# haoyuzhao123/CGRayTracing

Hardware: AMD Instinct MI355X
Metric: Mrays/sec (primary+secondary) at 1920x1080 spp=64 (higher is better)
Workload: dtype f64

## Files before the change

cgraytracing_amd/_capi.py:

```python
from __future__ import annotations

import ctypes as C
import os

import sys

_HERE = os.path.dirname(os.path.abspath(__file__))
CGRT_VERSION = 112
LIB_PATH = os.path.join(_HERE, "libcgrt.so")
if os.environ.get("CGRT_LIB"):
    if os.environ.get("CGRT_DEV_LIBS") == "1":
        LIB_PATH = os.environ["CGRT_LIB"]
        print("cgraytracing_amd: DEVELOPMENT library %s (CGRT_LIB + CGRT_DEV_LIBS=1)" % LIB_PATH, file=sys.stderr)
    else:
        print("cgraytracing_amd: CGRT_LIB ignored (set CGRT_DEV_LIBS=1 to load a development build)", file=sys.stderr)

CGRT_OK = 0
CGRT_NCOUNTERS = 8
CNT_RAYS, CNT_HITPOINTS, CNT_WAVE_ITERS, CNT_NODE_TESTS, CNT_TRI_TESTS = 0, 1, 2, 3, 4


class CgrtError(RuntimeError):
    def __init__(self, code, msg):
        super().__init__("libcgrt error %d: %s" % (code, msg))
        self.code = code


class Camera(C.Structure):
    _fields_ = [("cam", C.c_double * 3), ("half_width", C.c_double), ("focus_plane", C.c_double),
                ("lens_radius", C.c_double)]


class PosedCamera(C.Structure):
    _fields_ = [("base", Camera), ("origin", C.c_double * 3), ("right", C.c_double * 3), ("up", C.c_double * 3),
                ("forward", C.c_double * 3)]


class Grid(C.Structure):
    _fields_ = [("width", C.c_int32), ("height", C.c_int32), ("rows", C.c_int32), ("row_offset", C.c_int32),
                ("stripe_rows", C.c_int32), ("stripe_rank", C.c_int32), ("stripe_nranks", C.c_int32),
                ("spp", C.c_int32), ("sample_offset", C.c_int32), ("spp_total", C.c_int32),
                ("max_depth", C.c_int32), ("flags", C.c_int32), ("seed", C.c_uint64)]


GRID_STATS, GRID_ACCUMULATE, GRID_SPLIT_SAMPLES, GRID_NO_REORDER, GRID_FORCE_REORDER, GRID_HITPOINTS = 1, 2, 4, 8, 16, 32
GRID_NO_TILE_ORDER, GRID_DIFFUSE_TILES, GRID_NO_SPHERE_PAIRS, GRID_NO_SPHERE_MASKS = 64, 128, 256, 512
GRID_SAMPLE_RELAY, GRID_NO_SAMPLE_RELAY, GRID_SAMPLE_RELAY_4 = 1024, 2048, 4096
GRID_RELAY_MIRROR, GRID_RELAY_NO_MIRROR = 8192, 16384
GRID_RELAY_CHUNKS_FIRST, GRID_RELAY_MIRROR_FIRST, GRID_RELAY_INTERLEAVED, GRID_RELAY_ORDER_MASK = 32768, 65536, 98304, 98304
GRID_NO_LENS_STAGE, GRID_NO_SURE_TILES = 131072, 262144
GRID_RELAY_COST_START, GRID_NO_RELAY_COST_START, GRID_RELAY_BOOST, GRID_NO_RELAY_BOOST = 524288, 1048576, 2097152, 4194304
GRID_NO_LENS_TABLE, GRID_LENS_TABLE = 8388608, 16777216
GRID_NO_INSIDE_TRIPS = 33554432
GRID_POSED = 67108864


class Photons(C.Structure):
    _fields_ = [("light", C.c_double * 3), ("jitter", C.c_double), ("power", C.c_double), ("alpha", C.c_double),
                ("nphotons", C.c_int64), ("hashsize", C.c_int32), ("batch", C.c_int32), ("seed", C.c_uint64),
                ("initial_radius", C.c_double), ("pair_cap", C.c_int64)]


class PpmResult(C.Structure):
    _fields_ = [("image", C.c_void_p), ("rgb8", C.c_void_p), ("hp16", C.c_void_p), ("hp_cap", C.c_uint64),
                ("hp_count", C.c_uint64), ("n_events", C.c_uint64), ("n_pairs", C.c_uint64), ("n_batch_halvings", C.c_uint64),
                ("ms_eye", C.c_double),
                ("ms_table", C.c_double), ("ms_photons", C.c_double), ("ms_gather", C.c_double)]


class PpmSessionInfo(C.Structure):
    _fields_ = [("photons_done", C.c_int64), ("hp_count", C.c_uint64), ("n_events", C.c_uint64), ("n_pairs", C.c_uint64),
                ("n_batch_halvings", C.c_uint64), ("device_bytes", C.c_int64), ("ms_eye", C.c_double), ("ms_table", C.c_double),
                ("ms_photons", C.c_double), ("ms_last_add", C.c_double), ("ms_last_image", C.c_double)]


PPM_SESSION_NO_LOOKAHEAD = 1


class SppmSessionInfo(C.Structure):
    _fields_ = [("passes", C.c_int64), ("photons_done", C.c_int64), ("hp_count", C.c_uint64), ("n_events", C.c_uint64),
                ("n_pairs", C.c_uint64), ("n_batch_halvings", C.c_uint64), ("device_bytes", C.c_int64), ("ms_eye", C.c_double),
                ("ms_table", C.c_double), ("ms_photons", C.c_double), ("ms_update", C.c_double)]


class SceneStats(C.Structure):
    _fields_ = [("n_objects", C.c_int32), ("n_spheres", C.c_int32), ("n_planes", C.c_int32),
                ("n_meshes", C.c_int32), ("n_beziers", C.c_int32), ("n_textures", C.c_int32),
                ("n_trees", C.c_int32), ("committed", C.c_int32), ("n_triangles", C.c_int64),
                ("n_nodes", C.c_int64), ("device_bytes", C.c_int64), ("scene_bytes_fp64", C.c_int64)]


class BuildInfo(C.Structure):
    _fields_ = [("mode", C.c_int32), ("n_device_trees", C.c_int32), ("ms_host_build", C.c_double),
                ("ms_device_build", C.c_double), ("ms_commit", C.c_double)]


BUILD_HOST, BUILD_DEVICE = 0, 1


class Rays(C.Structure):
    _fields_ = [("n", C.c_int64), ("org3", C.c_void_p), ("dir3", C.c_void_p), ("keys", C.c_void_p),
                ("first_index", C.c_int64), ("seed", C.c_uint64), ("max_depth", C.c_int32), ("flags", C.c_int32)]


class RayResults(C.Structure):
    _fields_ = [("acc3", C.c_void_p), ("nhit", C.c_void_p), ("hit_obj", C.c_void_p), ("hit_t", C.c_void_p),
                ("hit_normal3", C.c_void_p)]


class HitAttributes(C.Structure):
    _fields_ = [("prim", C.c_void_p), ("uv2", C.c_void_p), ("color3", C.c_void_p), ("material2", C.c_void_p)]


class Occlusion(C.Structure):
    _fields_ = [("tmax", C.c_void_p), ("occluded", C.c_void_p)]


class Bounce(C.Structure):
    _fields_ = [("adj3", C.c_void_p), ("path", C.c_void_p), ("step", C.c_void_p), ("hit_obj", C.c_void_p), ("hit_t", C.c_void_p),
                ("pos3", C.c_void_p), ("normal3", C.c_void_p), ("value3", C.c_void_p), ("child_org3", C.c_void_p),
                ("child_dir3", C.c_void_p), ("child_adj3", C.c_void_p), ("child_path", C.c_void_p), ("child_keys", C.c_void_p),
                ("reserved", C.c_void_p * 2)]


class Wavefront(C.Structure):
    _fields_ = [("max_depth", C.c_int32), ("pad_", C.c_int32), ("min_adj", C.c_double), ("work_bytes", C.c_int64),
                ("acc3", C.c_void_p), ("nhit", C.c_void_p), ("hp9", C.c_void_p), ("hp_ray", C.c_void_p), ("hp_path", C.c_void_p),
                ("hp_cap", C.c_uint64), ("reserved", C.c_void_p * 2)]


WAVEFRONT_MAX_DEPTH = 31


class RayPixels(C.Structure):
    _fields_ = [("width", C.c_int32), ("rows", C.c_int32), ("spp", C.c_int32), ("pad_", C.c_int32), ("pixel", C.c_void_p)]

# ... 55 lines not shown
    "cgrt_ppm_session_create_rays": (C.c_int, [C.c_void_p, C.POINTER(Rays), C.POINTER(RayPixels), C.POINTER(Photons), C.c_int,
                                               C.POINTER(C.c_void_p)]),
    "cgrt_ppm_session_create_hitpoints": (C.c_int, [C.c_void_p, C.POINTER(Hitpoints), C.POINTER(Photons), C.c_int,
                                                    C.POINTER(C.c_void_p)]),
    "cgrt_ppm_session_destroy": (None, [C.c_void_p]),
    "cgrt_ppm_session_add_photons": (C.c_int, [C.c_void_p, C.c_int64]),
    "cgrt_ppm_session_add_photon_rays": (C.c_int, [C.c_void_p, C.POINTER(PhotonRays)]),
    "cgrt_photon_emit": (C.c_int, [C.POINTER(Photons), C.c_int64, C.c_int64, C.c_void_p, C.c_void_p, C.c_void_p, C.c_void_p, C.c_void_p,
                                   C.c_void_p]),
    "cgrt_photon_emit_host": (C.c_int, [C.POINTER(Photons), C.c_int64, C.c_int64, C.c_void_p, C.c_void_p, C.c_void_p, C.c_void_p,
                                        C.c_void_p]),
    "cgrt_photon_ray_events": (C.c_int, [C.c_void_p, C.POINTER(PhotonRays), C.c_uint64, C.c_int64, C.c_int, C.c_void_p, C.c_void_p]),
    "cgrt_ppm_session_image": (C.c_int, [C.c_void_p, C.c_void_p, C.c_void_p]),
    "cgrt_ppm_session_image_device": (C.c_int, [C.c_void_p, C.c_void_p, C.c_void_p, C.c_void_p]),
    "cgrt_ppm_session_hitpoints": (C.c_int, [C.c_void_p, C.c_void_p, C.c_uint64, C.POINTER(C.c_uint64)]),
    "cgrt_ppm_session_get_info": (C.c_int, [C.c_void_p, C.POINTER(PpmSessionInfo)]),
    "cgrt_sppm_session_create": (C.c_int, [C.c_void_p, C.c_int32, C.c_int32, C.c_int32, C.c_int32, C.POINTER(Photons), C.c_int32,
                                           C.POINTER(C.c_void_p)]),
    "cgrt_sppm_session_destroy": (None, [C.c_void_p]),
    "cgrt_sppm_session_pass_grid": (C.c_int, [C.c_void_p, C.POINTER(Camera), C.POINTER(Grid), C.c_int64]),
    "cgrt_sppm_session_pass_rays": (C.c_int, [C.c_void_p, C.POINTER(Rays), C.c_void_p, C.c_int64]),
    "cgrt_sppm_session_image": (C.c_int, [C.c_void_p, C.c_void_p, C.c_void_p]),
    "cgrt_sppm_session_image_device": (C.c_int, [C.c_void_p, C.c_void_p, C.c_void_p, C.c_void_p]),
    "cgrt_sppm_session_pixels": (C.c_int, [C.c_void_p, C.c_void_p]),
    "cgrt_sppm_session_last_hitpoints": (C.c_int, [C.c_void_p, C.c_void_p, C.c_uint64, C.POINTER(C.c_uint64)]),
    "cgrt_sppm_session_get_info": (C.c_int, [C.c_void_p, C.POINTER(SppmSessionInfo)]),
    "cgrt_sppm_update_host": (C.c_int, [C.c_double, C.c_double, C.c_void_p, C.c_double, C.c_void_p, C.c_double, C.c_void_p]),
    "cgrt_sppm_check_host": (C.c_int, [C.c_int32, C.c_int32, C.c_int32, C.c_int32, C.POINTER(Photons), C.c_int32, C.POINTER(Grid)]),
    "cgrt_tonemap_rgb8": (C.c_int, [C.c_int, C.c_void_p, C.c_int, C.c_int, C.c_void_p]),
    "cgrt_write_png": (C.c_int, [C.c_char_p, C.c_int, C.c_int, C.c_void_p]),
    "cgrt_photon_events": (C.c_int, [C.c_void_p, C.POINTER(Photons), C.c_int, C.c_int64, C.c_int32, C.c_void_p,
                                     C.c_void_p]),
    "cgrt_scene_bvh_dump": (C.c_int, [C.c_void_p, C.c_int, C.POINTER(C.c_int32), C.c_void_p, C.c_void_p]),
    "cgrt_scene_bvh_order": (C.c_int, [C.c_void_p, C.c_int, C.POINTER(C.c_int32), C.c_void_p]),
    "cgrt_scene_wide_dump": (C.c_int, [C.c_void_p, C.c_int, C.POINTER(C.c_int32), C.POINTER(C.c_int32), C.c_void_p, C.c_void_p]),
    "cgrt_lens_samples": (C.c_int, [C.c_uint64, C.c_void_p, C.c_void_p, C.c_int, C.c_double, C.c_void_p]),
    "cgrt_surface_colors": (C.c_int, [C.c_void_p, C.c_int, C.c_void_p, C.c_int, C.c_void_p]),
    "cgrt_trace_grid_variant": (C.c_int, [C.c_void_p, C.POINTER(Camera), C.POINTER(Grid), C.c_char_p, C.c_size_t]),
    "cgrt_scene_last_tile_order": (C.c_int, [C.c_void_p, C.c_void_p, C.c_void_p, C.c_void_p, C.c_int64, C.POINTER(C.c_int64)]),
    "cgrt_scene_last_sphere_masks": (C.c_int, [C.c_void_p, C.c_void_p, C.c_int64, C.POINTER(C.c_int64)]),
    "cgrt_scene_last_sure_tiles": (C.c_int, [C.c_void_p, C.c_void_p, C.c_int64, C.POINTER(C.c_int64)]),
    "cgrt_scene_last_sample_relay": (C.c_int, [C.c_void_p, C.POINTER(C.c_int64), C.POINTER(C.c_int32), C.POINTER(C.c_int64)]),
    "cgrt_scene_last_relay_form": (C.c_int, [C.c_void_p, C.POINTER(C.c_int32), C.POINTER(C.c_int32)]),
    "cgrt_scene_last_eye_launches": (C.c_int, [C.c_void_p, C.c_void_p, C.c_int64, C.POINTER(C.c_int64)]),
    "cgrt_relay_start_host": (C.c_int, [C.c_int32, C.c_int32, C.c_int32, C.c_int64, C.c_int32, C.c_int64, C.c_int64, C.c_int64, C.c_void_p,
                                        C.c_void_p, C.c_int32, C.c_int32, C.c_void_p, C.c_int64, C.POINTER(C.c_int64)]),
    "cgrt_scene_last_relay_start": (C.c_int, [C.c_void_p, C.c_void_p, C.c_int64, C.c_void_p, C.c_int64, C.POINTER(C.c_int64),
                                              C.POINTER(C.c_int64), C.POINTER(C.c_int32)]),
    "cgrt_scene_last_relay_boost": (C.c_int, [C.c_void_p, C.POINTER(C.c_int64), C.POINTER(C.c_int32), C.POINTER(C.c_int64), C.POINTER(C.c_uint64),
                                              C.POINTER(C.c_int32), C.POINTER(C.c_int32), C.POINTER(C.c_int32), C.c_void_p, C.c_int64]),
    "cgrt_relay_boost_host": (C.c_int, [C.c_int32, C.c_int32, C.c_int32, C.c_int64, C.c_int32, C.c_int64, C.c_int64, C.c_int64, C.c_void_p,
                                        C.c_void_p, C.c_int32, C.c_int32, C.c_int32, C.c_int32, C.c_int64, C.c_int32, C.c_int32, C.c_int32,
                                        C.c_void_p, C.c_int64, C.c_void_p, C.c_int64, C.POINTER(C.c_int64), C.POINTER(C.c_int64),
                                        C.POINTER(C.c_uint64)]),
    "cgrt_scene_last_lens_stage": (C.c_int, [C.c_void_p, C.POINTER(C.c_int64), C.POINTER(C.c_int64)]),
    "cgrt_scene_last_lens_table": (C.c_int, [C.c_void_p, C.POINTER(C.c_int64), C.POINTER(C.c_int64), C.POINTER(C.c_int32)]),
    "cgrt_scene_last_tile_order_reused": (C.c_int, [C.c_void_p, C.POINTER(C.c_int32)]),
    "cgrt_trace_grid_diffuse_variant": (C.c_int, [C.c_void_p, C.c_void_p, C.c_void_p, C.c_char_p, C.c_size_t]),
    "cgrt_scene_last_diffuse_tiles": (C.c_int, [C.c_void_p, C.POINTER(C.c_int64)]),
    "cgrt_scene_last_inkernel_diffuse_tiles": (C.c_int, [C.c_void_p, C.POINTER(C.c_int64)]),
    "cgrt_trace_rays": (C.c_int, [C.c_void_p, C.POINTER(Rays), C.POINTER(RayResults), C.c_void_p, C.c_void_p]),
    "cgrt_trace_rays_host": (C.c_int, [C.c_void_p, C.POINTER(Rays), C.POINTER(RayResults), C.c_void_p]),
    "cgrt_ray_hit_attributes": (C.c_int, [C.c_void_p, C.POINTER(Rays), C.c_void_p, C.c_void_p, C.POINTER(HitAttributes), C.c_void_p]),
    "cgrt_ray_hit_attributes_host": (C.c_int, [C.c_void_p, C.POINTER(Rays), C.c_void_p, C.c_void_p, C.POINTER(HitAttributes)]),
    "cgrt_trace_rays_variant": (C.c_int, [C.c_void_p, C.POINTER(Rays), C.POINTER(RayResults), C.c_char_p, C.c_size_t]),
    "cgrt_trace_rays_hitpoints": (C.c_int, [C.c_void_p, C.POINTER(Rays), C.c_void_p, C.c_uint64, C.POINTER(C.c_uint64)]),
    "cgrt_occlusion_rays": (C.c_int, [C.c_void_p, C.POINTER(Rays), C.POINTER(Occlusion), C.c_void_p, C.c_void_p]),
    "cgrt_occlusion_rays_host": (C.c_int, [C.c_void_p, C.POINTER(Rays), C.POINTER(Occlusion), C.c_void_p]),
    "cgrt_occlusion_rays_variant": (C.c_int, [C.c_void_p, C.POINTER(Rays), C.c_char_p, C.c_size_t]),
    "cgrt_bounce_rays": (C.c_int, [C.c_void_p, C.POINTER(Rays), C.POINTER(Bounce), C.c_void_p, C.c_void_p]),
    "cgrt_bounce_rays_host": (C.c_int, [C.c_void_p, C.POINTER(Rays), C.POINTER(Bounce), C.c_void_p]),
    "cgrt_bounce_rays_variant": (C.c_int, [C.c_void_p, C.POINTER(Rays), C.c_char_p, C.c_size_t]),
    "cgrt_wavefront_rays": (C.c_int, [C.c_void_p, C.POINTER(Rays), C.POINTER(Wavefront), C.c_void_p, C.POINTER(C.c_uint64), C.c_void_p]),
    "cgrt_wavefront_rays_host": (C.c_int, [C.c_void_p, C.POINTER(Rays), C.POINTER(Wavefront), C.c_void_p, C.POINTER(C.c_uint64)]),
    "cgrt_wavefront_rays_variant": (C.c_int, [C.c_void_p, C.POINTER(Rays), C.c_char_p, C.c_size_t]),
    "cgrt_scene_last_wavefront": (C.c_int, [C.c_void_p, C.POINTER(C.c_int64), C.POINTER(C.c_int64), C.POINTER(C.c_int32)]),
    "cgrt_scene_last_wavefront_rays": (C.c_int, [C.c_void_p, C.c_void_p]),
    "cgrt_camera_rays": (C.c_int, [C.POINTER(Camera), C.POINTER(Grid), C.c_void_p, C.c_void_p, C.c_void_p, C.c_void_p]),
    "cgrt_camera_rays_host": (C.c_int, [C.POINTER(Camera), C.POINTER(Grid), C.c_void_p, C.c_void_p, C.c_void_p]),
    "cgrt_intersect_rays": (C.c_int, [C.c_void_p, C.c_int, C.c_void_p, C.c_void_p, C.c_void_p, C.c_int,
                                      C.c_void_p, C.c_void_p, C.c_void_p]),
    "cgrt_math_probe": (C.c_int, [C.c_int, C.c_int, C.c_void_p, C.c_int64, C.c_void_p]),
    "cgrt_scene_inside_spheres": (C.c_int, [C.c_void_p, C.c_void_p, C.c_void_p, C.c_void_p, C.c_int32, C.POINTER(C.c_int32)]),
    "cgrt_inside_probe": (C.c_int, [C.c_void_p, C.c_int, C.c_void_p, C.c_int64, C.c_void_p]),
}

_lib = None


def lib():
    global _lib
    if _lib is None:
        if not os.path.exists(LIB_PATH):
            raise ImportError(
                "cgraytracing_amd: %s not found -- build the HIP library first "
                "(make -C cgraytracing_amd/csrc, or __graft_entry__.build()). There is no CPU fallback." % LIB_PATH)
        try:
            import torch
        except ImportError:
            pass
        L = C.CDLL(LIB_PATH)
        for name, (res, args) in SIGNATURES.items():
            fn = getattr(L, name)
            fn.restype = res
            fn.argtypes = args
        if L.cgrt_version() != CGRT_VERSION:
            raise ImportError("cgraytracing_amd: %s is ABI version %d, this binding needs %d -- rebuild it (make -C cgraytracing_amd/csrc)"
                              % (LIB_PATH, L.cgrt_version(), CGRT_VERSION))
        _lib = L
    return _lib


def check(rc):
    if rc < 0:
        raise CgrtError(rc, lib().cgrt_last_error().decode("utf-8", "replace"))
    return rc
```

cgraytracing_amd/csrc/cgrt_build.cpp:

```cpp
#include "cgrt_build.h"

#include <algorithm>
#include <atomic>
#include <chrono>
#include <future>
#include <thread>
#include <unordered_map>
#include <cmath>
#include <cstdio>
#include <cstdlib>
#include <cstring>

namespace cgrt {

namespace {

inline double hi3(double a, double b, double c) { return (a > b && a > c) ? a : (b > c ? b : c); }
inline double lo3(double a, double b, double c) { return (a < b && a < c) ? a : (b < c ? b : c); }
inline float round_down(double v) {
    float f = (float)v;
    return ((double)f > v) ? std::nextafterf(f, -INFINITY) : f;
}
inline float round_up(double v) {
    float f = (float)v;
// ... 929 lines not shown
        tr.lenx = t.lenx;
        tr.leny = t.leny;
        tr.isbump = t.isbump ? 1 : 0;
        L.texels.insert(L.texels.end(), t.rgb.begin(), t.rgb.end());
        L.texs.push_back(tr);
    }
    return L;
}

void scene_traits(const HostScene &H, const std::vector<TreeRec> &trees, const CommitKnobs &k, DeviceScene &d) {
    const std::vector<ObjRec> &objs = H.objs;
    d.n_objs = (int32_t)objs.size();
    d.n_lds = std::max(0, std::min({d.n_objs, kLdsObjsMax, k.lds_objs}));
    d.n_trees = (int32_t)trees.size();
    d.n_texs = (int32_t)H.textures.size();
    d.n_beziers = (int32_t)H.beziers.size();
    d.n_cover = (int32_t)(H.cover.size() / 4);
    d.has_wide = 0;
    for (const TreeRec &tr : trees)
        if (tr.nwide > 0) d.has_wide = 1;
    d.has_mesh = trees.empty() ? 0 : 1;
    d.has_bezier = H.beziers.empty() ? 0 : 1;
    d.cached_tree = -1;
    d.cached_nodes = 0;
    for (size_t t = 0; t < trees.size(); t++)
        if (trees[t].nnodes > 0 && trees[t].nnodes <= kNodeCache) {
            d.cached_tree = (int32_t)t;
            d.cached_nodes = trees[t].nnodes;
            break;
        }
    d.all_spheres = 1;
    d.has_glass = 0;
    for (const ObjRec &o : objs) {
        if (o.kind != KIND_SPHERE) d.all_spheres = 0;
        if (!(o.transp < kEps)) d.has_glass = 1;
    }
    {
        int n_mesh = 0, at = -1;
        for (size_t i = 0; i < objs.size(); i++)
            if (objs[i].kind == KIND_MESH) { n_mesh++; at = (int)i; }
        d.prim_obj = -1;
        if (n_mesh == 1 && H.beziers.empty() && objs[(size_t)at].transp < kEps && objs[(size_t)at].tree >= 0 &&
            trees[(size_t)objs[(size_t)at].tree].nwide > 0 && at < d.n_lds)
            d.prim_obj = at;
        d.prim_finish = d.prim_obj >= 0 ? 1 : 0;
        for (const ObjRec &o : objs)
            if (o.kind == KIND_PLANE && o.tree >= 0) d.prim_finish = 0;
    }
    bool planes_plain = true, special = false, plane_trees = false;
    for (const ObjRec &o : objs) {
        const bool diffuse = o.refl < kEps && o.transp < kEps;
        if (o.kind == KIND_PLANE && !diffuse) planes_plain = false;
        if (o.kind == KIND_PLANE && o.tree >= 0) plane_trees = true;
        if (o.kind == KIND_MESH || o.kind == KIND_BEZIER || (o.kind == KIND_SPHERE && !diffuse)) special = true;
    }
    d.light_ok = (planes_plain && special && !d.all_spheres) ? 1 : 0;
    d.single_ray = (planes_plain && !special) ? 1 : 0;
    d.light_trees = plane_trees ? 1 : 0;
    d.light_hf_only = plane_trees ? 1 : 0;
    for (const ObjRec &o : objs)
        if (o.kind == KIND_PLANE && o.tree >= 0 && !(o.transp < kEps && trees[(size_t)o.tree].hfield >= 0)) d.light_hf_only = 0;
    d.prun_begin = d.prun_end = 0;
    if (!k.no_plane_run) {
        auto eligible = [&](int j) { return objs[(size_t)j].kind == KIND_PLANE && objs[(size_t)j].axis >= 0 && objs[(size_t)j].tree < 0; };
        int b = 0;
        while (b < d.n_lds && objs[(size_t)b].kind == KIND_PLANE && !eligible(b)) b++;
        int j = b;
        while (j < d.n_lds && eligible(j)) j++;
        if (j - b >= 3) {
            d.prun_begin = b;
            d.prun_end = j;
        }
    }
    d.inside = InsideTrait{};
    if (d.all_spheres && d.n_objs == d.n_lds && d.n_objs <= kInsideSpheresMax) {
        std::vector<InsideBall> balls;
        std::vector<double> transp;
        for (const ObjRec &o : objs) {
            balls.push_back(InsideBall{{o.a[0], o.a[1], o.a[2]}, o.s0});
            transp.push_back(o.transp);
        }
        d.inside = inside_trait(balls.data(), transp.data(), d.n_objs, true);
    }
}

}
```

cgraytracing_amd/csrc/cgrt_build.h:

```cpp
#ifndef CGRT_BUILD_H
#define CGRT_BUILD_H
#include <cstdint>
#include <string>
#include <vector>

#include "cgrt_types.h"

namespace cgrt {

struct HostTree {
    std::vector<double> tri9;
    std::vector<int32_t> node_lr_size;
    std::vector<double> bbox;
    std::vector<int32_t> leaf_ids;
    std::vector<NodeRec> nodes;
    std::vector<TriRec> tris;
    std::vector<NodeRec> tboxes;
    std::vector<NodeRec> bvh;
    int32_t bvh_nodes = 0;
    bool tri_level = false;
    std::vector<OTriRec> otris;
    std::vector<WideNodeRec> wide;
    int32_t wide_stack = 0;
    void build_bvh(bool opaque);
    bool is_hfield = false;
    HFieldRec hfield{};
    std::vector<HCellRec> hcells;
    std::vector<HCellY> hcell_y;
    void build(bool opaque = false, bool with_bvh = true);
    void build_hfield(int nx, int nz, double x0, double z0, double hx, double hz);
    int dev_kind = 0;
    int64_t dev_ntri = 0;
    int dev_tex = -1;
    double dev_plane_y = 0;
    int dev_obj = -1;
    size_t dev_cover_at = 0;
    int32_t dev_nwide = 0;
    bool dev_balanced = false;
};
int64_t ref_node_count(int64_t n);

struct HostTexture {
    std::vector<uint8_t> rgb;
    int rows = 0, cols = 0;
    double n[3], p[3], lenx = 0, leny = 0;
    bool isbump = false;
};

struct HostScene {
    std::vector<ObjRec> objs;
    std::vector<HostTree> trees;
    std::vector<HostTexture> textures;
    std::vector<BezierRec> beziers;
    std::vector<BezSlabRec> bez_slabs;
    std::vector<double> cover;
    std::string error;
    int build_mode = 0;
    double host_build_ms = 0;

    int add_sphere(const double c[3], double r, const double sc[3], double refl, double transp);
    int add_texture(const uint8_t *rgb, int rows, int cols, const double n[3], const double p[3], double lx,
                    double ly, int isbump);
    int add_plane(const double p[3], const double n[3], const double sc[3], double refl, double transp, int tex);
    int add_mesh_file(const char *file, double a, const double b[3], const double sc[3], double refl,
                      double transp, int type);
    int add_mesh_triangles(const double *tri9, int ntri, const double sc[3], double refl, double transp, int type);
    int add_bezier(const double *cp3, int ncp, const double pos[3], const double sc[3], double refl, double transp);
};

bool load_mesh_file(const char *file, double a, const double b[3], int type, std::vector<double> &tri9,
                    std::string &err);


enum AuxPriority { AUX_LOWEST, AUX_SAME, AUX_HIGH };
struct CommitKnobs {
    bool ref_tree = false;
    int lds_objs = kLdsObjsMax;
    bool no_plane_run = false;
    bool no_bezier_cull = false;
    AuxPriority aux_priority = AUX_LOWEST;
};
CommitKnobs commit_knobs();

float tree_bmax(double max_abs);

struct SceneLayout {
    std::vector<NodeRec> nodes;
    std::vector<TriRec> tris;
    std::vector<OTriRec> otris;
    std::vector<NodeRec> tboxes;
    std::vector<WideNodeRec> wnodes;
    std::vector<HCellRec> hcells;
    std::vector<HCellY> hcell_y;
    std::vector<uint8_t> texels;
    std::vector<TexRec> texs;
    std::vector<HFieldRec> hfields;
    std::vector<TreeRec> trees;
    size_t room_tris = 0, room_otris = 0, room_wnodes = 0, room_hcells = 0;
    int n_dev_trees = 0;
};
SceneLayout scene_layout(const HostScene &H, const CommitKnobs &k);

void scene_traits(const HostScene &H, const std::vector<TreeRec> &trees, const CommitKnobs &k, DeviceScene &d);

}
#endif
```

cgraytracing_amd/csrc/cgrt_eye.hpp:

```cpp
#ifndef CGRT_EYE_HPP
#define CGRT_EYE_HPP
#include "cgrt_lens_stage.h"
#include "cgrt_scene_walk.hpp"
#include "cgrt_sphere_mask.h"
#include "cgrt_sure_first.h"
#include "cgrt_variants.h"

struct Pending {
    V3 o, d, adj;
    int32_t depth_left;
    uint32_t path;
};

#ifndef CGRT_DIFF_WAVES
#define CGRT_DIFF_WAVES 8
#endif
#ifndef CGRT_DIFF_DOF_WAVES
#define CGRT_DIFF_DOF_WAVES 6
#endif
static constexpr int kDiffWaves = CGRT_DIFF_WAVES, kDiffDofWaves = CGRT_DIFF_DOF_WAVES;

__host__ __device__ __forceinline__ void lens_disc(uint64_t k_smp, double &sx, double &sy) {
    uint64_t ctr = k_smp;
    while (true) {
        ctr += kGolden;
        const uint64_t z = fin64(ctr);
        const double ux = div_rand_max((uint32_t)(z >> 33)), uy = div_rand_max((uint32_t)((z >> 2) & 0x7fffffffu));
        sx = ux * 2.0 - 1;
        sy = uy * 2.0 - 1;
        if (sx * sx + sy * sy < 1) break;
    }
}

__device__ __forceinline__ V3 pose_v(const GridParams &g, const V3 &p) {
    V3 w;
    pose_point(g, p.x, p.y, p.z, w.x, w.y, w.z);
    return w;
}

struct HitpointSink {
    double *rec;
    unsigned long long *count;
    unsigned long long cap;
};

template <int NT>
__device__ __forceinline__ bool wave_has_tile(const GridParams &g, int tile_block, int tile_grid) {
    using TG = TileGeom<NT>;
    const int wave = threadIdx.x >> 6;
    const int wtiles_x = (g.W + kWaveTileW - 1) / kWaveTileW, wtiles_y = (g.rows + kWaveTileH - 1) / kWaveTileH;
    int tile_x, tile_y;
    if (tile_grid < 0) {
        const int tiles_x = (g.W + TG::W - 1) / TG::W;
        tile_x = tile_block % tiles_x;
        tile_y = tile_block / tiles_x;
    } else {
        const int tile_blocks = tile_grid / g.chunks;
        if (!tile_of_block(g, tile_block % tile_blocks, tile_x, tile_y, TG::W, TG::H)) return false;
    }
    const int wx = tile_x * (TG::W / kWaveTileW) + (NT == 256 ? (wave & 1) : 0);
    const int wy = tile_y * (TG::H / kWaveTileH) + (NT == 256 ? (wave >> 1) : 0);
    if (!(wx < wtiles_x && wy < wtiles_y)) return false;
    if (g.hidx && g.hidx[wy * wtiles_x + wx] >= 0) return false;
    if (g.light && (g.light[wy * wtiles_x + wx] != 0) != (g.light_mode != 0)) return false;
    return true;
}

struct RelayWg {
    int slot = -1, chunk = 0, s0 = 0, s1 = 0, boost = 0;
};
struct RelayForm {
    unsigned char *area;
    size_t cap;
    int k, slots;
};
template <bool COST>
__device__ __forceinline__ RelayForm relay_form(const GridParams &g, const RelayWg &rw) {
    if (COST && rw.boost) return RelayForm{g.relay + g.relay_boost_off, (size_t)g.boost_cap, g.boost_k, g.boost_slots};
    return RelayForm{g.relay, (size_t)g.relay_cap, g.relay_k, g.relay_slots};
}

template <bool TREES, bool BEZ, bool DOF, bool GLASS, bool SPH, bool STATS, bool HPS, int NT, bool HEAVY, bool SPILL = false, bool HFONLY = false,
          bool DIFF = false, bool PAIR = false, bool PARK = false, bool LSTAGE = false, bool COST = false, bool LTAB = false, bool POSE = false>
__device__ __forceinline__ void trace_grid_body(const DeviceScene &sc, const GridParams &g, float *__restrict__ rgb,
                                                uint32_t *__restrict__ nhit_out, unsigned long long *__restrict__ counters,
                                                const HitpointSink &hps, int tile_block, int tile_grid, const RelayWg rw = RelayWg{},
                                                const uint64_t *__restrict__ lens_row = nullptr) {
    using TG = TileGeom<NT>;
    static_assert(!LTAB || (PAIR && DOF && !LSTAGE), "LTAB: the thin-lens PAIR variants' full and parking bodies");
    static_assert(!PARK || (PAIR && NT == kRelayThreads), "PARK: a relayed tile's later chunks");
    static_assert(!DIFF || (SPH && !GLASS && !HPS && !HEAVY && !STATS && !SPILL), "DIFF: the sphere loop, first hits only");
    static_assert(!PAIR || (SPH && GLASS && !HPS && !HEAVY && !STATS && !SPILL), "PAIR: the glass sphere variants of the tile order");
    static_assert(!LSTAGE || (DIFF && DOF && !PAIR), "LSTAGE: the thin-lens terminal-diffuse body inside a PAIR launch");
    static_assert(!COST || PAIR, "COST: the PAIR variants with a start table");
    static_assert(!POSE || (!DIFF && !PAIR && !LSTAGE && !LTAB), "POSE: no body of the tile order, whose tests stand in the built-in frame");
    static_assert(!LSTAGE || lens_batch_lds(NT) <= (size_t)kLdsLevels * pending_level_bytes(NT), "the lens batches fit the PAIR launch's pending-ray levels");
    const long long tl_t0 = g.timeline ? wall_clock64() : 0;
    if (!HEAVY && !g.timeline) {
        if (!__syncthreads_or((int)wave_has_tile<NT>(g, tile_block, tile_grid))) return;
    }
    constexpr size_t level_bytes = pending_level_bytes(NT), stack_bytes = (size_t)kLdsLevels * level_bytes;
    constexpr bool WALK = TREES && !HFONLY;
    {
        constexpr WgLds chk = wg_lds(wg_ask_trace(NT, TREES, BEZ, GLASS, SPILL, HFONLY), 3, 5, true);
        static_assert(chk.pending == 0 && chk.objs == (GLASS ? stack_bytes : 0) && chk.staging - chk.objs == 3 * sizeof(ObjRec) &&
                          chk.bez - chk.staging == (SPILL ? (NT / 64) * sizeof(ObjRec) : 0) &&
                          chk.nodes - chk.bez == (BEZ ? (NT / 64) * sizeof(BezLds) : 0) &&
                          chk.wstack - chk.nodes == (WALK ? 5 * sizeof(NodeRec) : 0) && chk.has.nodes == WALK &&
                          chk.has.wstack == (WALK && !GLASS && !BEZ),
                      "trace_grid_body's carve-up and cgrt_wg_lds.h");
    }
    extern __shared__ __align__(16) unsigned char lds_raw[];
    ObjRec *lobjs = reinterpret_cast<ObjRec *>(lds_raw + (GLASS ? stack_bytes : 0));
    unsigned char *lrest = reinterpret_cast<unsigned char *>(lobjs + sc.n_lds);
    LdsAux aux;
    if (SPILL) {
        aux.spill = reinterpret_cast<ObjRec *>(lrest) + (threadIdx.x >> 6);
        lrest += (NT / 64) * sizeof(ObjRec);
    }
    aux.bl = BEZ ? reinterpret_cast<volatile BezLds *>(lrest) + (threadIdx.x >> 6) : nullptr;
    if (BEZ) lrest += (NT / 64) * sizeof(BezLds);
    NodeRec *lnodes = reinterpret_cast<NodeRec *>(lrest);
    aux.lnodes = (WALK && sc.cached_tree >= 0) ? lnodes : nullptr;
    aux.wstack = (WALK && !GLASS && !BEZ && sc.has_wide)
                     ? reinterpret_cast<uint2 *>(lrest + ((sc.cached_tree >= 0 ? (size_t)sc.cached_nodes * sizeof(NodeRec) : 0)))
                     : nullptr;
    if (WALK && sc.cached_tree >= 0) {
        const uint4 *src = reinterpret_cast<const uint4 *>(sc.nodes + sc.trees[sc.cached_tree].node_begin);
        uint4 *dst = reinterpret_cast<uint4 *>(lnodes);
        const int n16 = sc.cached_nodes * (int)(sizeof(NodeRec) / 16);
        for (int k = threadIdx.x; k < n16; k += NT) dst[k] = src[k];
    }

    {
        const uint4 *src = reinterpret_cast<const uint4 *>(sc.objs);
        uint4 *dst = reinterpret_cast<uint4 *>(lobjs);
        const int n16 = sc.n_lds * (int)(sizeof(ObjRec) / 16);
        for (int k = threadIdx.x; k < n16; k += NT) dst[k] = src[k];
    }
    __syncthreads();
    const long long cost_t0 = g.probe ? (long long)clock64() : 0;

    const int wave = threadIdx.x >> 6, lane = threadIdx.x & 63;
    const int wtiles_x = (g.W + kWaveTileW - 1) / kWaveTileW, wtiles_y = (g.rows + kWaveTileH - 1) / kWaveTileH;
    const V3 camorg = mk(g.cam[0], g.cam[1], g.cam[2]);
    const V3 camw = POSE ? pose_v(g, camorg) : camorg;
    constexpr bool heavy = HEAVY;
    const unsigned long long lanes_below = (1ull << lane) - 1ull;

    int wx = 0, wy = 0, chunk = 0, s_end = 0;
    bool have_tile = false;
    int w = 0, j = 0, h = 0;
    bool live = false;
    V3 pdir = mk(0, 0, 1), pof = mk(0, 0, 0);
    uint64_t k_pix = 0;
    auto set_pixel = [&](int lx, int ly) {
        w = wx * kWaveTileW + lx;
        j = wy * kWaveTileH + ly;
        h = global_row(g, j);
        live = have_tile && (w < g.W) && (j < g.rows) && (h < g.H);
        const double px = (2.0 * ((double)w / g.W) - 1) * g.half_width;
        const double py = (2.0 * ((double)h / g.H) - 1) * g.half_width * g.H / g.W;
        pdir = normalized(mk(px, py, 0) - camorg);
        pof = pdir * ((g.focus_plane - camorg.z) / pdir.z) + camorg;
        if (POSE) {
            pof = pose_v(g, pof);
            pdir = normalized(pose_v(g, mk(px, py, 0)) - camw);
        }
        k_pix = pixel_key(g.seed, (uint64_t)h * (uint64_t)g.W + (uint64_t)w);
    };
    if (!heavy) {
        const int nb = tile_block;
        int tile_x, tile_y;
        if (tile_grid < 0) {
            const int tiles_x = (g.W + TG::W - 1) / TG::W;
            tile_x = nb % tiles_x;
            tile_y = nb / tiles_x;
        } else {
            const int tile_blocks = tile_grid / g.chunks;
            chunk = nb / tile_blocks;
            if (!tile_of_block(g, nb % tile_blocks, tile_x, tile_y, TG::W, TG::H)) return;
        }
        wx = tile_x * (TG::W / kWaveTileW) + (NT == 256 ? (wave & 1) : 0);
        wy = tile_y * (TG::H / kWaveTileH) + (NT == 256 ? (wave >> 1) : 0);
        have_tile = wx < wtiles_x && wy < wtiles_y;
        if (have_tile && g.hidx && g.hidx[wy * wtiles_x + wx] >= 0) have_tile = false;
        if (have_tile && g.light && (g.light[wy * wtiles_x + wx] != 0) != (g.light_mode != 0)) have_tile = false;
        s_end = (g.chunks > 1) ? ((chunk + 1) * g.chunk_spp < g.spp ? (chunk + 1) * g.chunk_spp : g.spp) : (PAIR && rw.slot >= 0 ? rw.s1 : g.spp);
        set_pixel(lane & 15, lane >> 4);
    }
    const bool masked = DIFF && g.wmask != nullptr;
    uint32_t smask = 0u;
    if (masked) {
        smask = load_uniform(g.wmask + __builtin_amdgcn_readfirstlane(have_tile ? wy * wtiles_x + wx : 0));
        if (sc.n_lds < 32) smask &= (1u << sc.n_lds) - 1u;
    }
    uint32_t sure = (uint32_t)kSureNone;
    if (DIFF && g.wsure != nullptr && have_tile) {
        const uint32_t wt = (uint32_t)__builtin_amdgcn_readfirstlane(wy * wtiles_x + wx);
        sure = (load_uniform(reinterpret_cast<const uint32_t *>(g.wsure) + (wt >> 2)) >> ((wt & 3u) * 8u)) & 0xffu;
        if (sure >= (uint32_t)sc.n_lds) sure = (uint32_t)kSureNone;
    }
    uint64_t k_smp = 0;

    double acc_r = 0, acc_g = 0, acc_b = 0;
    uint32_t my_hits = 0, my_rays = 0, my_nodes = 0, my_tris = 0, wave_iters = 0;
    uint32_t hp_seq = 0;

    Pending deep[2];
    Pending sib;
    bool sib_valid = false;
    unsigned char *lslot = lds_raw;
    int sp = 0;
    int s = (g.chunks > 1) ? chunk * g.chunk_spp : (PAIR && rw.slot >= 0 ? rw.s0 : 0);
    double *park = nullptr;
    uint32_t park_n = 0;
    if (PARK) {
        const RelayForm rf = relay_form<COST>(g, rw);
        park = reinterpret_cast<double *>(rf.area + relay_layout(rf.cap, rf.k, rf.slots).rvals) +
               ((size_t)rw.slot * (size_t)(rf.k - 1) + (size_t)(rw.chunk - 1)) * (size_t)rf.slots * (3 * NT) + threadIdx.x;
    }
    bool have = false;
    V3 o = camorg, d = pdir, adj = mk(1, 1, 1);
    int depth_left = 0;
    uint32_t path = 1;
    int unit_next = 0, unit_end = 0, hrank = 0;
    int unit_pix = 0, unit_smp = 0, unit_rank = 0;
    bool unit_open = false;
    constexpr bool PRE = HEAVY && TREES && !BEZ && !STATS && !SPILL;
    bool pre_valid = false;
    double pre_len = 0;
    int32_t pre_tri = -1;

    const bool staging = LSTAGE && g.lens_batch != 0;
    uint64_t *const lens_slot = reinterpret_cast<uint64_t *>(lrest) + threadIdx.x;
    static_assert(lens_slot_at(1, 0, NT) == NT * sizeof(uint64_t) && lens_slot_at(0, 1, NT) == sizeof(uint64_t), "lens_slot's strides");
    int batch_first = 0, batch_end = 0;
    auto stage_lens = [&](int first, int count) {
        uint32_t rejected = 0u;
        for (int b = 0; b < count; b++) {
            const LensSlot a = lens_stage_first(k_pix, (uint64_t)(g.sample_offset + first + b));
            lens_slot[b * NT] = a.v;
            rejected |= a.done ? 0u : (1u << b);
        }
        if (!live) rejected = 0u;
        while (__ballot(rejected != 0u) != 0ull) {
            if (rejected != 0u) {
                const int b = __ffs((int)rejected) - 1;
                const LensSlot a = lens_stage_retry(lens_slot[b * NT]);
                lens_slot[b * NT] = a.v;
                if (a.done) rejected &= rejected - 1u;
            }
        }
        batch_first = first;
        batch_end = first + count;
    };
    uint64_t z_next = 0;
    if (LTAB && s < s_end) z_next = lens_row[(uint32_t)s * (uint32_t)NT + threadIdx.x];
    auto start_sample = [&](int smp) {
        if (LTAB) {
            double sx, sy;
            lens_point(z_next, sx, sy);
            o = camorg + mk(sx, sy, 0) * g.lens_radius;
            d = normalized(pof - o);
            k_smp = 0;
            if (smp + 1 < s_end) z_next = lens_row[(uint32_t)(smp + 1) * (uint32_t)NT + threadIdx.x];
        } else if (LSTAGE && staging) {
            double sx, sy;
            lens_point(lens_slot[(smp - batch_first) * NT], sx, sy);
            o = camorg + mk(sx, sy, 0) * g.lens_radius;
            d = normalized(pof - o);
            k_smp = 0;
        } else if (DOF) {
            k_smp = sample_key(k_pix, (uint64_t)(g.sample_offset + smp));
            double sx, sy;
            lens_disc(k_smp, sx, sy);
            o = camorg + mk(sx, sy, 0) * g.lens_radius;
            if (POSE) o = pose_v(g, o);
            d = normalized(pof - o);
        } else {
            k_smp = sample_key(k_pix, (uint64_t)(g.sample_offset + smp));
            o = POSE ? camw : camorg;
            d = pdir;
// ... 395 lines not shown
        for (int off = 32; off > 0; off >>= 1) {
            r += __shfl_xor(r, off);
            hh += __shfl_xor(hh, off);
            if (STATS) {
                nn += __shfl_xor(nn, off);
                tt += __shfl_xor(tt, off);
            }
        }
        if (lane == 0 && (r | (unsigned long long)wave_iters) != 0ull) {
            atomicAdd(&counters[CGRT_CNT_RAYS], r);
            atomicAdd(&counters[CGRT_CNT_HITPOINTS], hh);
            atomicAdd(&counters[CGRT_CNT_WAVE_ITERS], (unsigned long long)wave_iters);
            if (STATS) {
                atomicAdd(&counters[CGRT_CNT_NODE_TESTS], nn);
                atomicAdd(&counters[CGRT_CNT_TRI_TESTS], tt);
            }
        }
    }
}

__device__ __forceinline__ unsigned long long *wg_counters_begin(unsigned long long *wg, const unsigned long long *counters) {
    if (!counters) return nullptr;
    if (threadIdx.x < CGRT_NCOUNTERS) wg[threadIdx.x] = 0ull;
    __syncthreads();
    return wg;
}
__device__ __forceinline__ void wg_counters_end(const unsigned long long *wg, unsigned long long *counters) {
    if (!counters) return;
    __syncthreads();
    if (threadIdx.x < CGRT_NCOUNTERS && wg[threadIdx.x] != 0ull) atomicAdd(&counters[threadIdx.x], wg[threadIdx.x]);
}

template <bool TREES, bool BEZ, bool DOF, bool GLASS, bool SPH, bool STATS, bool HPS = false, int NT = 256, bool SPILL = false, bool HFONLY = false,
          bool DIFF = false, bool PAIR = false, bool START = false, bool LTAB = false, bool POSE = false>
__global__ __launch_bounds__(NT, DIFF ? (DOF ? kDiffDofWaves : kDiffWaves) : BEZ ? kBezWaves : ((TREES && !HFONLY) ? kTreeWaves : 4)) void trace_grid_kernel(DeviceScene sc, GridParams g, float *__restrict__ rgb,
                                                             uint32_t *__restrict__ nhit_out,
                                                             unsigned long long *__restrict__ counters,
                                                             HitpointSink hps = HitpointSink{nullptr, nullptr, 0}) {
    int tile_block = (int)blockIdx.x, tile_grid = (int)gridDim.x;
    unsigned entry = blockIdx.x;
    RelayWg rw;
    if (!POSE && g.tile_order) {
        if (g.tile_order == kOrderFull || g.tile_order == kOrderDiffuse) {
            const unsigned first_diffuse = load_uniform(g.plan + 3);
            if (g.tile_order == kOrderDiffuse) entry += first_diffuse;
            if (g.tile_order == kOrderDiffuse ? entry >= load_uniform(g.plan + kOrderClasses) : entry >= first_diffuse) return;
        } else if (PAIR && g.relay_k > 1) {
            const unsigned n_tiles = load_uniform(g.plan + kOrderClasses);
            const unsigned n01 = load_uniform(g.plan + 2), n012 = load_uniform(g.plan + 3);
            RelayBlock rb{n_tiles, 0, false};
            bool tabled = false;
            unsigned b = blockIdx.x, bslot = 0u;
            if (START && g.relay_start_at != 0u) {
                const unsigned n_split = relay_split_entries(n01, n012, (unsigned)g.relay_cap, g.relay_extent);
                const unsigned t0 = n012 + ((unsigned)g.relay_k - 1u) * n_split;
                const unsigned items = g.relay_boost_at != 0u ? load_uniform(g.plan + g.relay_boost_at + kBoostItems) : t0;
                tabled = b < items;
                if (tabled) {
                    rb = relay_start_block(load_uniform(g.plan + g.relay_start_at + b), n_split);
                    if (g.relay_boost_at != 0u && rb.split) bslot = load_uniform(g.plan + g.relay_boost_at + kBoostHead + rb.entry);
                    if (rb.chunk >= (bslot != 0u ? g.boost_k : g.relay_k) || bslot > (unsigned)g.boost_cap) return;
                } else {
                    b -= items - t0;
                }
            }
            if (!tabled) rb = relay_block_ordered(b, (unsigned)g.relay_k, n01, n012, n_tiles, (unsigned)g.relay_cap, g.relay_extent, g.relay_order);
            entry = rb.entry;
            if (entry >= n_tiles) return;
            if (rb.split) {
                const int cs = START && bslot != 0u ? g.boost_chunk_spp : g.relay_chunk_spp;
                rw.slot = START && bslot != 0u ? (int)(bslot - 1u) : (int)entry;
                rw.boost = START && bslot != 0u ? 1 : 0;
                rw.chunk = rb.chunk;
                rw.s0 = relay_first_sample(rb.chunk, cs);
                rw.s1 = relay_end_sample(rb.chunk, cs, g.spp);
            }
        }
        tile_block = (int)load_uniform(g.border + entry);
        tile_grid = -1;
    }
    __shared__ unsigned long long wg_cnt[CGRT_NCOUNTERS];
    unsigned long long *wc = wg_counters_begin(wg_cnt, counters);
    if (PAIR && g.tile_order == kOrderAllDiffuse && entry >= load_uniform(g.plan + 3))
        trace_grid_body<false, false, DOF, false, true, false, false, NT, false, false, false, true, false, false, DOF>(sc, g, rgb, nhit_out, wc, hps, tile_block, tile_grid);
    else if (LTAB && g.lens_table != nullptr && entry < (unsigned)g.lens_table_cap && entry < load_uniform(g.plan + 3)) {
        const uint64_t *lens_row = g.lens_table + (size_t)entry * (size_t)g.lens_table_spp * NT;
        if (rw.chunk > 0)
            trace_grid_body<TREES, BEZ, DOF, GLASS, SPH, STATS, HPS, NT, false, SPILL, HFONLY, DIFF, PAIR, PAIR, false, START, LTAB>(sc, g, rgb, nhit_out, wc, hps, tile_block, tile_grid, rw, lens_row);
        else
            trace_grid_body<TREES, BEZ, DOF, GLASS, SPH, STATS, HPS, NT, false, SPILL, HFONLY, DIFF, PAIR, false, false, START, LTAB>(sc, g, rgb, nhit_out, wc, hps, tile_block, tile_grid, rw, lens_row);
    } else if (PAIR && rw.chunk > 0)
        trace_grid_body<TREES, BEZ, DOF, GLASS, SPH, STATS, HPS, NT, false, SPILL, HFONLY, DIFF, PAIR, PAIR, false, START>(sc, g, rgb, nhit_out, wc, hps, tile_block, tile_grid, rw);
    else
        trace_grid_body<TREES, BEZ, DOF, GLASS, SPH, STATS, HPS, NT, false, SPILL, HFONLY, DIFF, PAIR, false, false, START, false, POSE>(sc, g, rgb, nhit_out, wc, hps, tile_block, tile_grid, rw);
    wg_counters_end(wg_cnt, counters);
}
template <bool TREES, bool BEZ, bool DOF, bool GLASS, bool SPH, bool STATS, int NT = 256, bool POSE = false>
__global__ __launch_bounds__(NT, BEZ ? kBezWaves : (TREES ? kSchedTreeWaves : 4)) void trace_grid_sched_kernel(DeviceScene sc, GridParams g,
                                                                                         float *__restrict__ rgb,
                                                                                         uint32_t *__restrict__ nhit_out,
                                                                                         unsigned long long *__restrict__ counters) {
    const HitpointSink none{nullptr, nullptr, 0};
    const bool heavy_first = (int)blockIdx.x < g.heavy_blocks;
    __shared__ unsigned long long wg_cnt[CGRT_NCOUNTERS];
    unsigned long long *wc = wg_counters_begin(wg_cnt, counters);
    if (NT == 64) {
        if (heavy_first)
            trace_grid_body<TREES, BEZ, DOF, GLASS, SPH, STATS, false, NT, true, false, false, false, false, false, false, false, false, POSE>(sc, g, rgb, nhit_out, wc, none, 0, 1);
        else
            trace_grid_body<TREES, BEZ, DOF, GLASS, SPH, STATS, false, NT, false, false, false, false, false, false, false, false, false, POSE>(
                sc, g, rgb, nhit_out, wc, none, (int)blockIdx.x - g.heavy_blocks, (int)gridDim.x - g.heavy_blocks);
        wg_counters_end(wg_cnt, counters);
        return;
    }
    const bool queued = g.border != nullptr;
    __shared__ unsigned tile_entry;
    for (int phase = 0; phase < 2; phase++) {
        if ((phase == 0) == heavy_first) {
            if (queued || heavy_first)
                trace_grid_body<TREES, BEZ, DOF, GLASS, SPH, STATS, false, NT, true, false, false, false, false, false, false, false, false, POSE>(sc, g, rgb, nhit_out, wc, none, 0, 1);
        } else {
            const unsigned n_entries = queued ? load_uniform(g.plan + 3) : (heavy_first ? 0u : 1u);
            unsigned served = 0;
            while (true) {
                unsigned e = served++;
                if (queued) {
                    __syncthreads();
                    if (threadIdx.x == 0) tile_entry = atomicAdd(&g.plan[4], 1u);
                    __syncthreads();
                    e = tile_entry;
                }
                if (e >= n_entries) break;
                trace_grid_body<TREES, BEZ, DOF, GLASS, SPH, STATS, false, NT, false, false, false, false, false, false, false, false, false, POSE>(
                    sc, g, rgb, nhit_out, wc, none, queued ? (int)g.border[e] : (int)blockIdx.x - g.heavy_blocks,
                    queued ? -1 : (int)gridDim.x - g.heavy_blocks);
            }
        }
    }
    wg_counters_end(wg_cnt, counters);
}

__global__ void finalize_chunks_kernel(GridParams g, float *__restrict__ rgb, uint32_t *__restrict__ nhit_out) {
    const size_t npx = (size_t)g.rows * g.W;
    const size_t px = (size_t)blockIdx.x * blockDim.x + threadIdx.x;
    if (px >= npx) return;
    if (g.hidx) {
        const int wtiles_x = (g.W + kWaveTileW - 1) / kWaveTileW;
        if (g.hidx[(int)((px / g.W) / kWaveTileH) * wtiles_x + (int)((px % g.W) / kWaveTileW)] >= 0) return;
    }
    double r = 0, gg = 0, b = 0;
    uint32_t hits = 0;
    for (int c = 0; c < g.chunks; c++) {
        const size_t q = (size_t)c * npx + px;
        r += g.partial[3 * q + 0];
        gg += g.partial[3 * q + 1];
        b += g.partial[3 * q + 2];
        if (g.partial_nhit) hits += g.partial_nhit[q];
    }
    const float fr = (float)(r * g.inv_spp_total), fg = (float)(gg * g.inv_spp_total), fb = (float)(b * g.inv_spp_total);
    float *dst = rgb + 3 * px;
    if (g.accumulate) {
        dst[0] += fr; dst[1] += fg; dst[2] += fb;
    } else {
        dst[0] = fr; dst[1] = fg; dst[2] = fb;
    }
    if (nhit_out) nhit_out[px] = hits;
}
// ... 431 lines not shown
            }
        }
    }
    const float fr = (float)(r * g.inv_spp_total), fg = (float)(gg * g.inv_spp_total), fb = (float)(b * g.inv_spp_total);
    float *dst = rgb + ((size_t)j * g.W + w) * 3;
    if (g.accumulate) {
        dst[0] += fr; dst[1] += fg; dst[2] += fb;
    } else {
        dst[0] = fr; dst[1] = fg; dst[2] = fb;
    }
    if (nhit_out) nhit_out[(size_t)j * g.W + w] = hits;
}

__global__ void intersect_rays_kernel(DeviceScene sc, int obj, const double *__restrict__ org,
                                      const double *__restrict__ dir, const unsigned long long *__restrict__ keys,
                                      int n, int32_t *__restrict__ hit,
                                      double *__restrict__ len, double *__restrict__ nrm) {
    __shared__ BezLds bl;
    const int i = blockIdx.x * blockDim.x + threadIdx.x;
    const bool on = i < n;
    const int ii = on ? i : 0;
    uint32_t a = 0, b = 0;
    const V3 o = ld3(org + 3 * ii), d = ld3(dir + 3 * ii);
    DeviceScene one = sc;
    one.prun_begin = one.prun_end = 0;
    RayKey rk{keys ? keys[ii] : 0ull, 1, true, 0u};
    const LdsAux aux{&bl, nullptr};
    SceneHit h = intersect_scene<true, true, false, false>(sc.objs + obj, 1, 1, one, o, d, rk, on, aux, a, b);
    if (!on) return;
    hit[i] = h.id >= 0 ? 1 : 0;
    len[i] = h.t;
    nrm[3 * i] = h.n.x;
    nrm[3 * i + 1] = h.n.y;
    nrm[3 * i + 2] = h.n.z;
}

__device__ __forceinline__ V3 surface_color(const DeviceScene &sc, const ObjRec &ob, V3 P) {
    V3 f = ld3(ob.col);
    if (ob.kind == KIND_PLANE && ob.tex >= 0) {
        V3 c;
        if (texture_color(sc.texs[ob.tex], sc.texels, P, c)) f = c;
    }
    return f;
}

__global__ void surface_colors_kernel(DeviceScene sc, int obj, const double *__restrict__ pts, int n, double *__restrict__ out) {
    const int i = blockIdx.x * blockDim.x + threadIdx.x;
    if (i >= n) return;
    const V3 f = surface_color(sc, sc.objs[obj], ld3(pts + 3 * i));
    out[3 * i] = f.x;
    out[3 * i + 1] = f.y;
    out[3 * i + 2] = f.z;
}

__global__ void math_probe_kernel(int op, const double *__restrict__ in, long long n, double *__restrict__ out) {
    const long long i = (long long)blockIdx.x * blockDim.x + threadIdx.x;
    if (i >= n) return;
    if (op == CGRT_PROBE_SQRT) {
        out[i] = sqrt_cr(in[i]);
    } else if (op == CGRT_PROBE_NORMALIZED) {
        const V3 v = normalized(ld3(in + 3 * i));
        out[3 * i] = v.x;
        out[3 * i + 1] = v.y;
        out[3 * i + 2] = v.z;
    } else if (op == CGRT_PROBE_SPHERE_LEN) {
        const double *p = in + 10 * i;
        out[i] = sphere_len(ld3(p), p[3], ld3(p + 4), ld3(p + 7));
    } else {
        const double *p = in + 14 * i;
        sphere_len_pair(ld3(p), p[3], ld3(p + 4), p[7], ld3(p + 8), ld3(p + 11), out[2 * i], out[2 * i + 1]);
    }
}

__global__ void inside_loop_probe_kernel(DeviceScene sc, InsideTrait guarded, const double *__restrict__ in, long long n, double *__restrict__ out) {
    const long long i = (long long)blockIdx.x * blockDim.x + threadIdx.x;
    if (i >= n) return;
    const V3 o = ld3(in + 6 * i), d = ld3(in + 6 * i + 3);
    RayKey rk{0, 1, false, 0u};
    LdsAux aux;
    aux.bl = nullptr;
    aux.lnodes = nullptr;
    uint32_t nn = 0, nt = 0;
    sc.inside = InsideTrait{};
    const SceneHit a = intersect_scene<false, false, true, false, false, false, false, false, true>(sc.objs, sc.n_lds, sc.n_objs, sc, o, d, rk, true, aux, nn, nt);
    sc.inside = guarded;
    const SceneHit b = intersect_scene<false, false, true, false, false, false, false, false, true>(sc.objs, sc.n_lds, sc.n_objs, sc, o, d, rk, true, aux, nn, nt);
    bool took = false;
    for (int k = 0; k < kInsideMax && k < guarded.n && !took; k++)
        took = __ballot(!starts_inside(o, ld3(sc.objs[guarded.idx[k]].a), guarded.rin2[k])) == 0ull;
    out[5 * i] = a.t;
    out[5 * i + 1] = (double)a.id;
    out[5 * i + 2] = b.t;
    out[5 * i + 3] = (double)b.id;
    out[5 * i + 4] = took ? 1.0 : 0.0;
}

#endif
```

cgraytracing_amd/csrc/cgrt_frame.h:

```cpp
#ifndef CGRT_FRAME_H
#define CGRT_FRAME_H
#include <algorithm>
#include <cmath>
#include <cstddef>
#include <cstdint>
#include <cstdio>
#include <cstdlib>
#include <string>

#include "../../include/cgrt.h"
#include "cgrt_lens_stage.h"
#include "cgrt_relay.h"

struct GridParams {
    int32_t W, H, rows, row_offset, stripe_rows, stripe_rank, stripe_nranks;
    int32_t spp, sample_offset, max_depth;
    int32_t accumulate;
    int32_t xcd_tiles;
    int32_t chunks, chunk_spp;
    double *partial;
    uint32_t *partial_nhit;
    const unsigned char *light;
    int32_t light_mode, tile_order;
    const uint32_t *wmask;
    const uint32_t *order;
    const uint32_t *border;
    uint32_t *cost;
    const int32_t *hidx;
    uint32_t *plan;
    double *dvals;
    unsigned char *dcnt;
    double *pconst;
    int32_t probe, heavy_blocks, items_per_tile, units_per_item, maxhp;
    const double *prim_len;
    const int32_t *prim_tri;
    int32_t prim_obj;
    int32_t prim_done;
    int32_t pw_refill, pw_rounds;
    unsigned long long *timeline;
    double inv_spp_total;
    uint64_t seed;
    double cam[3], half_width, focus_plane, lens_radius;
    unsigned char *relay;
    int32_t relay_k, relay_chunk_spp, relay_cap, relay_slots;
    int32_t relay_extent, relay_order;
    int32_t lens_batch;
    uint32_t relay_start_at;
    const unsigned char *wsure;
    uint64_t relay_boost_off;
    uint32_t relay_boost_at;
    int32_t boost_k, boost_chunk_spp, boost_cap, boost_slots, pad_boost_;
    const uint64_t *lens_table;
    int32_t lens_table_cap, lens_table_spp;
    double pose_origin[3], pose_right[3], pose_up[3], pose_forward[3];
    int32_t posed, pad_pose_;
};
static_assert(sizeof(GridParams) == 488, "GridParams is a kernel argument: its layout is fixed");
static_assert(offsetof(GridParams, pose_origin) == 384, "the pose is appended: no earlier field moves");

#if defined(__HIPCC__)
#define CGRT_HD __host__ __device__ __forceinline__
#else
#define CGRT_HD inline
#endif
CGRT_HD void pose_point(const GridParams &g, double x, double y, double z, double &wx, double &wy, double &wz) {
    wx = ((g.pose_origin[0] + g.pose_right[0] * x) + g.pose_up[0] * y) + g.pose_forward[0] * z;
    wy = ((g.pose_origin[1] + g.pose_right[1] * x) + g.pose_up[1] * y) + g.pose_forward[1] * z;
    wz = ((g.pose_origin[2] + g.pose_right[2] * x) + g.pose_up[2] * y) + g.pose_forward[2] * z;
}

static constexpr double kPoseTol = 1e-9;
inline const char *pose_error(const cgrt_camera *cam, const cgrt_grid *grid) {
    if (!(grid->flags & CGRT_GRID_POSED)) return nullptr;
    const cgrt_posed_camera *pc = reinterpret_cast<const cgrt_posed_camera *>(cam);
    const double *ax[3] = {pc->right, pc->up, pc->forward};
    for (int k = 0; k < 3; k++) {
        if (!std::isfinite(pc->origin[k])) return "posed camera: origin is not finite";
        for (int a = 0; a < 3; a++)
            if (!std::isfinite(ax[a][k])) return "posed camera: a basis vector is not finite";
    }
    const auto dot3 = [](const double *a, const double *b) { return a[0] * b[0] + a[1] * b[1] + a[2] * b[2]; };
    for (int a = 0; a < 3; a++)
        if (!(std::fabs(std::sqrt(dot3(ax[a], ax[a])) - 1.0) <= kPoseTol)) return "posed camera: right, up and forward must have length 1 (within 1e-9)";
    for (int a = 0; a < 3; a++)
        if (!(std::fabs(dot3(ax[a], ax[(a + 1) % 3])) <= kPoseTol)) return "posed camera: right, up and forward must be orthogonal (dot products within 1e-9)";
    return nullptr;
}

inline const char *look_at_camera(const double eye[3], const double target[3], const double up_hint[3], double fov_x_deg,
                                  double focus_distance, double lens_radius, cgrt_posed_camera *out) {
    for (int k = 0; k < 3; k++)
        if (!std::isfinite(eye[k]) || !std::isfinite(target[k]) || !std::isfinite(up_hint[k])) return "cgrt_look_at: eye, target and up_hint must be finite";
    if (!(fov_x_deg > 0 && fov_x_deg < 180)) return "cgrt_look_at: fov_x_deg must lie in (0, 180)";
    if (!(focus_distance > 0) || !std::isfinite(focus_distance)) return "cgrt_look_at: focus_distance must be positive";
    if (!(lens_radius >= 0) || !std::isfinite(lens_radius)) return "cgrt_look_at: lens_radius must be >= 0";
// ... 98 lines not shown
            r += cam.lens_radius * std::max(std::fabs(1 - s_lo), std::fabs(1 - s_hi));
        }
        const double vx = sp.s[i][0] - cam.cam[0], vy = sp.s[i][1] - cam.cam[1], vz = sp.s[i][2] - cam.cam[2];
        if (!(std::sqrt(vx * vx + vy * vy + vz * vz) > r)) return true;
    }
    return false;
}
static constexpr int kWaveTileW = 16, kWaveTileH = 4;
static constexpr int kXcds = 8, kSuperW = 4, kSuperH = 4, kSuperTiles = kSuperW * kSuperH;

inline int tile_grid_blocks(int W, int rows, bool xcd_tiles, int tile_w = kTileW, int tile_h = kTileH) {
    const int tiles_x = (W + tile_w - 1) / tile_w, tiles_y = (rows + tile_h - 1) / tile_h;
    if (!xcd_tiles) return tiles_x * tiles_y;
    const int sx = (tiles_x + kSuperW - 1) / kSuperW, sy = (tiles_y + kSuperH - 1) / kSuperH;
    const int nsuper = sx * sy;
    return ((nsuper + kXcds - 1) / kXcds) * kXcds * kSuperTiles;
}

inline GridParams grid_params(const cgrt_camera *cam, const cgrt_grid *grid) {
    GridParams g{};
    g.W = grid->width;
    g.H = grid->height;
    g.rows = grid->rows;
    g.row_offset = grid->row_offset;
    g.stripe_rows = grid->stripe_rows;
    g.stripe_rank = grid->stripe_rank;
    g.stripe_nranks = grid->stripe_nranks;
    g.spp = grid->spp;
    g.sample_offset = grid->sample_offset;
    g.max_depth = grid->max_depth;
    g.accumulate = (grid->flags & CGRT_GRID_ACCUMULATE) ? 1 : 0;
    g.inv_spp_total = 1.0 / (double)grid->spp_total;
    g.seed = grid->seed;
    for (int k = 0; k < 3; k++) g.cam[k] = cam->cam[k];
    g.half_width = cam->half_width;
    g.focus_plane = cam->focus_plane;
    g.lens_radius = cam->lens_radius;
    g.chunks = 1;
    g.chunk_spp = grid->spp;
    g.items_per_tile = 1;
    g.units_per_item = 256;
    g.maxhp = 16;
    g.prim_obj = -1;
    g.pw_refill = 16;
    g.pw_rounds = 8;
    g.pose_right[0] = g.pose_up[1] = g.pose_forward[2] = 1.0;
    if (grid->flags & CGRT_GRID_POSED) {
        const cgrt_posed_camera *pc = reinterpret_cast<const cgrt_posed_camera *>(cam);
        for (int k = 0; k < 3; k++) {
            g.pose_origin[k] = pc->origin[k];
            g.pose_right[k] = pc->right[k];
            g.pose_up[k] = pc->up[k];
            g.pose_forward[k] = pc->forward[k];
        }
        g.posed = 1;
    }
    return g;
}

struct EyeKnobs {
    bool force_reorder = false;
    long long defer_bytes = 0;
    int heavy_div = 32, units_per_item = 256;
    bool no_primwalk = false, pw_no_finish = false;
    int pw_refill = 16, pw_rounds = 8;
    int lds_pad = 0;
    bool no_hfonly = false, no_tile_queue = false, plan_dump = false;
    bool no_sure_tiles = false;
    bool no_order_reuse = false;
    int relay_chunks = kRelayDefaultChunks;
    long long relay_tiles = 0;
    int relay_mirror = -1;
    int relay_order = -1;
    int relay_start = -1;
    int relay_probe_spp = kRelayProbeSpp;
    bool relay_boost_off = false;
    uint32_t relay_boost_num = kRelayBoostNum, relay_boost_den = kRelayBoostDen;
    long long relay_boost_tiles = -1;
    int lens_stage = -1;
    int lens_table = -1;
    long long lens_table_bytes = 0;
    bool lens_table_bytes_set = false;
    bool no_inside_trips = false;
    const char *timeline_file = nullptr;
};
inline const char *env_str(const char *name) { const char *e = std::getenv(name); return e ? e : ""; }
inline bool env_on(const char *name) { const char *e = env_str(name); return *e && *e != '0'; }
inline int env_positive(const char *name, int def) { const int v = std::atoi(env_str(name)); return v > 0 ? v : def; }
inline int relay_order_named(const char *e) {
    const std::string v(e);
    if (v == "chunks_first" || v == "0") return kRelayChunksFirst;
    if (v == "mirror_first" || v == "1") return kRelayMirrorFirst;
    if (v == "interleaved" || v == "2") return kRelayInterleaved;
    return -1;
}
inline int relay_start_named(const char *e) {
    const std::string v(e);
    if (v == "list" || v == "0") return kRelayStartList;
    if (v == "cost" || v == "1") return kRelayStartCost;
    return -1;
}
inline bool relay_boost_named(const char *e, bool &off, uint32_t &num, uint32_t &den) {
    const std::string v(e);
    if (v.empty()) return true;
    if (v == "off" || v == "0") {
        off = true;
        return true;
    }
    const size_t slash = v.find('/');
    if (slash == std::string::npos || slash == 0 || slash + 1 >= v.size()) return false;
    for (size_t i = 0; i < v.size(); i++)
        if (i != slash && (v[i] < '0' || v[i] > '9')) return false;
    if (slash > 6 || v.size() - slash - 1 > 6) return false;
    const unsigned long n = std::strtoul(v.c_str(), nullptr, 10), d = std::strtoul(v.c_str() + slash + 1, nullptr, 10);
    if (n > kRelayBoostMaxTerm || d < 1 || d > kRelayBoostMaxTerm) return false;
    num = (uint32_t)n;
    den = (uint32_t)d;
    return true;
}
static constexpr int kLensStageOff = 0, kLensStageLds = 1;
static constexpr int kLensStageDefault = kLensStageLds;
inline int lens_stage_named(const char *e) {
    const std::string v(e);
    if (v == "off" || v == "0") return kLensStageOff;
    if (v == "lds" || v == "1") return kLensStageLds;
    return -1;
}
static constexpr bool kLensTableAlways = false;
inline int lens_table_named(const char *e) {
    const std::string v(e);
    if (v == "off" || v == "0") return 0;
    if (v == "on" || v == "1") return 1;
    return -1;
}
inline EyeKnobs eye_knobs() {
    static const EyeKnobs once = [] {
        EyeKnobs k;
        k.force_reorder = env_on("CGRT_FORCE_REORDER");
        k.defer_bytes = std::atoll(env_str("CGRT_DEFER_BYTES"));
        k.heavy_div = env_positive("CGRT_HEAVY_DIV", 32);
        k.units_per_item = (env_positive("CGRT_UNITS_PER_ITEM", 256) + 63) / 64 * 64;
        k.no_primwalk = env_on("CGRT_NO_PRIMWALK");
        k.pw_no_finish = env_on("CGRT_PW_NO_FINISH");
        k.pw_refill = env_positive("CGRT_PW_REFILL", 16);
        k.pw_rounds = env_positive("CGRT_PW_ROUNDS", 8);
        k.lds_pad = std::atoi(env_str("CGRT_LDS_PAD"));
        k.no_hfonly = env_on("CGRT_NO_HFONLY");
        k.no_tile_queue = env_on("CGRT_NO_TILE_QUEUE");
        k.plan_dump = env_on("CGRT_PLAN_DUMP");
        k.no_order_reuse = env_on("CGRT_NO_ORDER_REUSE");
        k.no_sure_tiles = env_on("CGRT_NO_SURE_TILES");
        k.relay_chunks = std::min(std::max(env_positive("CGRT_RELAY_CHUNKS", kRelayDefaultChunks), 2), kRelayMaxChunks);
        k.relay_tiles = std::atoll(env_str("CGRT_RELAY_TILES"));
        if (*env_str("CGRT_RELAY_MIRROR")) k.relay_mirror = env_on("CGRT_RELAY_MIRROR") ? 1 : 0;
        k.relay_order = relay_order_named(env_str("CGRT_RELAY_ORDER"));
        k.relay_start = relay_start_named(env_str("CGRT_RELAY_START"));
        if (k.relay_start < 0 && *env_str("CGRT_RELAY_START"))
            std::fprintf(stderr, "cgrt: CGRT_RELAY_START=%s names no start order of this library (list, cost): the default is used\n", env_str("CGRT_RELAY_START"));
        {
            const int ps = std::atoi(env_str("CGRT_RELAY_PROBE_SPP"));
            if (ps == 1 || ps == 2 || ps == 4) k.relay_probe_spp = ps;
        }
        k.lens_stage = lens_stage_named(env_str("CGRT_LENS_STAGE"));
        if (k.lens_stage < 0 && *env_str("CGRT_LENS_STAGE"))
            std::fprintf(stderr, "cgrt: CGRT_LENS_STAGE=%s names no form of this library (off, lds): the default is used\n", env_str("CGRT_LENS_STAGE"));
        k.lens_table = lens_table_named(env_str("CGRT_LENS_TABLE"));
        if (k.lens_table < 0 && *env_str("CGRT_LENS_TABLE"))
            std::fprintf(stderr, "cgrt: CGRT_LENS_TABLE=%s is neither off nor on: the default is used\n", env_str("CGRT_LENS_TABLE"));
        if (*env_str("CGRT_LENS_TABLE_BYTES")) {
            k.lens_table_bytes = std::max(std::atoll(env_str("CGRT_LENS_TABLE_BYTES")), 0ll);
            k.lens_table_bytes_set = true;
        }
        {
            const std::string v(env_str("CGRT_INSIDE_TRIPS"));
            k.no_inside_trips = v == "off" || v == "0";
            if (!v.empty() && !k.no_inside_trips && v != "on" && v != "1")
                std::fprintf(stderr, "cgrt: CGRT_INSIDE_TRIPS=%s is neither off nor on: the default is used\n", v.c_str());
        }
        return k;
    }();
    EyeKnobs k = once;
    k.timeline_file = *env_str("CGRT_TIMELINE_FILE") ? env_str("CGRT_TIMELINE_FILE") : nullptr;
    if (!relay_boost_named(env_str("CGRT_RELAY_BOOST"), k.relay_boost_off, k.relay_boost_num, k.relay_boost_den)) {
        static bool said = false;
        if (!said)
            std::fprintf(stderr, "cgrt: CGRT_RELAY_BOOST=%s is neither off nor a threshold num/den (integers, num <= %u, 1 <= den <= %u): the default is used\n",
                         env_str("CGRT_RELAY_BOOST"), kRelayBoostMaxTerm, kRelayBoostMaxTerm);
        said = true;
    }
    if (*env_str("CGRT_RELAY_BOOST_TILES")) k.relay_boost_tiles = std::max(std::atoll(env_str("CGRT_RELAY_BOOST_TILES")), 0ll);
    return k;
}

struct FrameInputs {
    cgrt_grid grid;
    cgrt_camera cam;
    bool sched, spill, stats, glass;
    int nt;
    bool has_mesh, has_bezier, prim_finish, light_ok;
    int prim_obj;
    EyeKnobs knobs;
    size_t mem_total;
    int n_cu, waves_per_simd;
    bool image = false, sph = false, pair = false;
    bool order_ok = false, aux_stream = false, all_spheres = false;
    int n_objs = 0, n_lds = 0;
    bool all_special = false;
    bool posed = false;
    cgrt_posed_camera posed_cam{};
};

struct ScratchLayout {
    Region partial{}, partial_nhit{}, cost{}, order{}, hidx{}, border{}, plan{}, light{}, dvals{}, dcnt{}, pconst{}, prim_len{}, prim_tri{};
    size_t total = 0;
    void place(GridParams &g, unsigned char *base, bool nhit) const {
        g.partial = partial.in<double>(base);
        g.partial_nhit = nhit ? partial_nhit.in<uint32_t>(base) : nullptr;
        g.cost = cost.in<uint32_t>(base);
        g.order = order.in<uint32_t>(base);
        g.hidx = hidx.in<int32_t>(base);
        g.border = border.in<uint32_t>(base);
        g.plan = plan.in<uint32_t>(base);
        g.light = light.in<unsigned char>(base);
        g.dvals = dvals.in<double>(base);
        g.dcnt = dcnt.in<unsigned char>(base);
        g.pconst = pconst.in<double>(base);
        g.prim_len = prim_len.in<double>(base);
        g.prim_tri = prim_tri.in<int32_t>(base);
    }
};

struct TileOrderPlan {
    bool on = false;
    enum Class3 { None, SecondLaunch, InKernel } class3 = None;
    bool masks = false;
    bool sure = false;
    int lens_stage = kLensStageOff;
    size_t lens_table_cap = 0, lens_table_bytes = 0;
    bool lens_table_always = false;
};

inline bool relay_engaged(int32_t flags, int32_t spp, size_t n_tiles, int n_cu) {
    if ((flags & CGRT_GRID_NO_SAMPLE_RELAY) || spp < 2 * kRelayMinChunkSpp) return false;
    return (flags & CGRT_GRID_SAMPLE_RELAY) || n_tiles >= (size_t)4 * (size_t)n_cu;
}

static constexpr int kRelayDefaultExtent = kRelayMirror, kRelayDefaultOrder = kRelayInterleaved;
struct RelayRule { int extent, order, start; bool boost; };
inline RelayRule relay_rule(int32_t f, const EyeKnobs &kn) {
    const bool asked = (f & CGRT_GRID_SAMPLE_RELAY) != 0;
    const int32_t order_flag = f & CGRT_GRID_RELAY_ORDER_MASK;
    const bool measured = !asked && !order_flag && kn.relay_order < 0;
    const bool names_start = (f & (CGRT_GRID_NO_RELAY_COST_START | CGRT_GRID_RELAY_COST_START)) || kn.relay_start >= 0;
    RelayRule r;
    r.extent = (f & CGRT_GRID_RELAY_MIRROR) ? kRelayMirror : (f & CGRT_GRID_RELAY_NO_MIRROR) ? kRelayGlass
               : kn.relay_mirror >= 0 ? (kn.relay_mirror ? kRelayMirror : kRelayGlass) : asked ? kRelayGlass : kRelayDefaultExtent;
    r.order = order_flag ? (order_flag == CGRT_GRID_RELAY_MIRROR_FIRST ? kRelayMirrorFirst : order_flag == CGRT_GRID_RELAY_INTERLEAVED ? kRelayInterleaved : kRelayChunksFirst)
              : kn.relay_order >= 0 ? kn.relay_order : asked ? kRelayChunksFirst : kRelayDefaultOrder;
    r.start = (f & CGRT_GRID_NO_RELAY_COST_START) ? kRelayStartList : (f & CGRT_GRID_RELAY_COST_START) ? kRelayStartCost
              : kn.relay_start >= 0 ? kn.relay_start : measured ? kRelayStartCost : kRelayStartList;
    r.boost = (f & CGRT_GRID_NO_RELAY_BOOST) ? false : (f & CGRT_GRID_RELAY_BOOST) ? true : !kn.relay_boost_off && !names_start && measured;
    return r;
}

struct RelayArea {
    int k = 0, chunk_spp = 0, slots = 0;
    size_t cap = 0, bytes = 0;
};
static constexpr int kRelayWgPerCu = 4;
struct RelayPlan {
    RelayArea base{1, 0, 0, 0, 0}, boost;
    int spp = 0, extent = kRelayGlass, order = kRelayChunksFirst;
    int start = kRelayStartList, probe_spp = 0;
    size_t start_words = 0, boost_words = 0;
    uint32_t num = 0, den = 1;
    int wg_slots = 0;
    bool relays() const { return base.k > 1; }
    bool boosts() const { return boost.k > base.k; }
    size_t boost_at() const { return align256(base.bytes); }
    size_t bytes() const { return boosts() ? boost_at() + boost.bytes : base.bytes; }
    size_t grid(size_t n_tiles, bool boosted) const { return relay_grid(n_tiles, base.k, base.cap) + (boosted ? boost_words : 0); }
    RelayBoost boost_rule() const {
        return boosts() ? RelayBoost{(uint32_t)boost.k, (uint32_t)boost.cap, boost.chunk_spp, num, den, (uint32_t)wg_slots} : RelayBoost{};
    }
    RelayItems items(uint32_t n01, uint32_t n012, uint32_t n_tiles) const {
        return RelayItems{(uint32_t)base.k, n01, n012, n_tiles, (uint32_t)base.cap, extent, base.chunk_spp, spp};
    }
    TileOrderLayout order_layout(size_t n_tiles, size_t n_wt, bool sure) const {
        return tile_order_layout(n_tiles, n_wt, sure, start_words, boost_words, base.cap, boost.k);
    }
    void place(GridParams &g, unsigned char *buf) const {
        g.relay = buf;
        g.relay_k = base.k;
        g.relay_chunk_spp = base.chunk_spp;
        g.relay_cap = (int32_t)base.cap;
        g.relay_slots = base.slots;
        g.relay_extent = extent;
        g.relay_order = order;
        if (!boosts()) return;
        g.relay_boost_off = boost_at();
        g.boost_k = boost.k;
        g.boost_chunk_spp = boost.chunk_spp;
        g.boost_cap = (int32_t)boost.cap;
        g.boost_slots = boost.slots;
    }
};
inline RelayPlan relay_plan(const cgrt_grid &gr, const EyeKnobs &kn, size_t n_tiles, int n_cu, size_t mem_total) {
    RelayPlan r;
    if (!relay_engaged(gr.flags, gr.spp, n_tiles, n_cu)) return r;
    const auto area = [&gr](const RelayChunks &c, size_t tiles, size_t budget, long long bound) {
        RelayArea a{c.k, c.chunk_spp, relay_slots(c.chunk_spp, gr.max_depth), 0, 0};
        a.cap = relay_cap(tiles, a.k, a.slots, budget, bound);
        a.bytes = relay_layout(a.cap, a.k, a.slots).total;
        return a;
    };
    const RelayChunks rc = relay_chunks(gr.spp, (gr.flags & CGRT_GRID_SAMPLE_RELAY_4) ? kRelayMaxChunks : kn.relay_chunks);
    const RelayArea base = rc.k > 1 ? area(rc, n_tiles, relay_budget(mem_total), kn.relay_tiles) : RelayArea{};
    if (base.cap == 0) return r;
    const RelayRule f = relay_rule(gr.flags, kn);
    r.base = base;
    r.spp = gr.spp, r.extent = f.extent, r.order = f.order;
    r.start = n_tiles < kRelayStartMaxTiles ? f.start : kRelayStartList;
    if (r.start != kRelayStartCost) return r;
    r.probe_spp = std::min(kn.relay_probe_spp, (int)gr.spp);
    r.start_words = relay_start_words(n_tiles, base.k, base.cap);
    const RelayChunks rb = relay_chunks(gr.spp, kRelayMaxChunks);
    if (rb.k <= rc.k || !f.boost || kn.relay_boost_tiles == 0) return r;
    const RelayArea boost = area(rb, base.cap, relay_boost_budget(mem_total, r.boost_at()), kn.relay_boost_tiles);
    if (boost.cap == 0) return r;
    r.boost = boost;
    r.boost_words = relay_boost_extra(base.k, boost.k, boost.cap);
    r.num = kn.relay_boost_num, r.den = kn.relay_boost_den;
    r.wg_slots = n_cu * kRelayWgPerCu;
    return r;
}

struct FramePlan {
    int chunks = 1, chunk_spp = 0;
    bool xcd_tiles = false;
    int maxhp = 1;
    int tile_blocks = 0;
    size_t grid_dim = 0;
    int wtiles_x = 0, wtiles_y = 0;
    size_t n_wt = 0, tile_bytes = 0, kmax = 0;
    bool use_prim = false;
    bool split_light = false, tile_queue = false, prim_done = false;
    int wave_slots = 0, items_per_tile = 1, heavy_blocks = 0;
    unsigned long long plan_div = 0;
    ScratchLayout scratch;
    TileOrderPlan order;
    RelayPlan relay;
};

inline FramePlan frame_plan(const FrameInputs &in, size_t kmax) {
    const cgrt_grid &gr = in.grid;
    const EyeKnobs &kn = in.knobs;
    FramePlan p;
    p.chunk_spp = gr.spp;
    p.xcd_tiles = !in.spill && in.has_mesh && !in.has_bezier;
    p.maxhp = in.glass ? 16 : 1;
    const size_t npx = (size_t)gr.rows * gr.width;
    if ((gr.flags & CGRT_GRID_SPLIT_SAMPLES) && gr.spp >= 32 && !in.spill) {
        int chunks = std::min(gr.spp / 16, 16);
        while (chunks > 1 && (size_t)chunks * npx * 28 > ((size_t)4 << 30)) chunks--;
        if (chunks > 1) {
            p.chunk_spp = (gr.spp + chunks - 1) / chunks;
            p.chunks = (gr.spp + p.chunk_spp - 1) / p.chunk_spp;
        }
    }
    const bool one_wave = in.nt == 64;
    const int waves_per_block = in.nt / 64;
    p.tile_blocks = one_wave ? tile_grid_blocks(gr.width, gr.rows, false, kWaveTileW, kWaveTileH)
                             : tile_grid_blocks(gr.width, gr.rows, p.xcd_tiles);
    p.grid_dim = (size_t)p.tile_blocks * p.chunks;
    TileOrderPlan &o = p.order;
    const bool split_asked = (gr.flags & CGRT_GRID_SPLIT_SAMPLES) != 0;
    o.on = in.image && p.chunks == 1 && !p.xcd_tiles && in.nt == kThreads && in.order_ok && !(gr.flags & CGRT_GRID_NO_TILE_ORDER) && !in.posed;
    if (o.on && !in.all_special) {
        if (in.sph && !in.spill && !in.stats && in.aux_stream && (gr.flags & CGRT_GRID_DIFFUSE_TILES) && !split_asked && !kn.timeline_file)
            o.class3 = TileOrderPlan::SecondLaunch;
        else if (in.pair)
            o.class3 = TileOrderPlan::InKernel;
    }
    o.masks = o.class3 != TileOrderPlan::None && in.all_spheres && in.n_objs <= kSphereMaskMax && in.n_objs == in.n_lds &&
              !(gr.flags & CGRT_GRID_NO_SPHERE_MASKS);
    o.sure = o.masks && !(gr.flags & CGRT_GRID_NO_SURE_TILES) && !kn.no_sure_tiles;
    if (o.class3 == TileOrderPlan::InKernel && in.cam.lens_radius > 0 && !(gr.flags & CGRT_GRID_NO_LENS_STAGE))
        o.lens_stage = kn.lens_stage >= 0 ? kn.lens_stage : kLensStageDefault;
    if (o.on && in.pair && o.class3 != TileOrderPlan::SecondLaunch && !split_asked)
        p.relay = relay_plan(gr, kn, (size_t)p.tile_blocks, in.n_cu, in.mem_total);
    const int lens_table = (gr.flags & CGRT_GRID_NO_LENS_TABLE) ? 0 : (gr.flags & CGRT_GRID_LENS_TABLE) ? 1 : kn.lens_table;
    if (o.on && in.pair && o.class3 != TileOrderPlan::SecondLaunch && !split_asked && in.cam.lens_radius > 0 && lens_table != 0) {
        const size_t budget = kn.lens_table_bytes_set ? (size_t)kn.lens_table_bytes : kLensTableBudget;
        o.lens_table_cap = lens_table_cap((size_t)p.tile_blocks, gr.spp, kThreads, budget);
        o.lens_table_bytes = lens_table_bytes(o.lens_table_cap, gr.spp, kThreads);
        o.lens_table_always = o.lens_table_cap > 0 && (lens_table > 0 || kLensTableAlways);
    }
    p.wtiles_x = (gr.width + kWaveTileW - 1) / kWaveTileW;
    p.wtiles_y = (gr.rows + kWaveTileH - 1) / kWaveTileH;
    p.n_wt = (size_t)p.wtiles_x * p.wtiles_y;
    p.use_prim = in.sched && in.prim_obj >= 0 && !kn.no_primwalk && !(gr.flags & CGRT_GRID_STATS) && !in.posed;
    const size_t units = (size_t)gr.spp * 64;
    const size_t vals = units * (size_t)p.maxhp * 3 * sizeof(double), cnt = (units + 7) & ~(size_t)7, pconst = 7 * 64 * sizeof(double),
                 plen = p.use_prim ? units * sizeof(double) : 0, ptri = p.use_prim ? units * sizeof(int32_t) : 0;
    p.tile_bytes = vals + cnt + pconst + plen + ptri;
    p.kmax = in.sched ? kmax : 0;

    ScratchLayout &L = p.scratch;
    size_t end = 0;
    const auto take = [&end](size_t bytes, bool used = true) { end += bytes; return Region{end - bytes, used ? bytes : 0}; };
    if (p.chunks > 1) {
        L.partial = take((size_t)p.chunks * npx * 3 * sizeof(double));
        L.partial_nhit = take((size_t)p.chunks * npx * sizeof(uint32_t));
    }
    L.total = end = align256(end);
    if (!in.sched) return p;
    const size_t np = (p.n_wt + 8) * sizeof(uint32_t), sched_bytes = align256(4 * np + 64 * sizeof(uint32_t) + align256(p.n_wt));
    L.total += sched_bytes + (p.kmax ? p.kmax * p.tile_bytes + 256 : 0);
    if (p.kmax == 0) return p;
    p.split_light = in.light_ok && p.chunks == 1 && !in.stats && !in.posed;
    p.tile_queue = p.chunks == 1 && !one_wave && !kn.no_tile_queue;
    p.prim_done = p.use_prim && in.prim_finish && !kn.pw_no_finish;
    p.wave_slots = in.n_cu * 4 * in.waves_per_simd;
    p.plan_div = (unsigned long long)p.wave_slots * (unsigned long long)kn.heavy_div;
    p.items_per_tile = (int)((units + kn.units_per_item - 1) / kn.units_per_item);
    const size_t fill = (size_t)p.wave_slots / waves_per_block;
    p.heavy_blocks = (int)std::min((p.kmax * (size_t)p.items_per_tile + waves_per_block - 1) / waves_per_block, fill);
    if (p.tile_queue) p.grid_dim = fill;
    const size_t sched_at = end;
    L.cost = take(np);
    L.order = take(np);
    L.hidx = take(np);
    L.border = take(np, p.tile_queue);
    L.plan = take(64 * sizeof(uint32_t));
    L.light = take(p.n_wt, p.split_light);
    end = sched_at + sched_bytes;
    L.dvals = take(p.kmax * vals);
    L.dcnt = take(p.kmax * cnt);
    L.pconst = take(p.kmax * pconst);
    L.prim_len = take(p.kmax * plen);
    L.prim_tri = take(p.kmax * ptri);
    return p;
}

inline size_t max_heavy_tiles(const FrameInputs &in) {
    if (!in.sched) return 0;
    const FramePlan p = frame_plan(in, 0);
    const size_t budget = in.knobs.defer_bytes > 0 ? (size_t)in.knobs.defer_bytes : std::min((size_t)12 << 30, in.mem_total / 8);
    return std::min(budget / p.tile_bytes, p.n_wt);
}

inline size_t fit_heavy_tiles(const FrameInputs &in, size_t kmax, size_t refused) {
    while (refused && kmax > 0 && frame_plan(in, kmax).scratch.total >= refused) kmax /= 2;
    return kmax;
}

inline GridParams frame_params(const FrameInputs &in, const FramePlan &p) {
    GridParams g = grid_params(in.posed ? &in.posed_cam.base : &in.cam, &in.grid);
    g.xcd_tiles = p.xcd_tiles ? 1 : 0;
    g.chunks = p.chunks;
    g.chunk_spp = p.chunk_spp;
    g.maxhp = p.maxhp;
    g.units_per_item = in.knobs.units_per_item;
    g.pw_refill = in.knobs.pw_refill;
    g.pw_rounds = in.knobs.pw_rounds;
    g.items_per_tile = p.items_per_tile;
    g.heavy_blocks = p.heavy_blocks;
    g.lens_batch = p.order.lens_stage == kLensStageLds ? 1 : 0;
    g.lens_table_cap = (int32_t)p.order.lens_table_cap;
    g.lens_table_spp = p.order.lens_table_cap ? in.grid.spp : 0;
    if (p.heavy_blocks > 0 && p.use_prim) {
        g.prim_obj = in.prim_obj;
        g.prim_done = p.prim_done ? 1 : 0;
    }
    return g;
}

#endif
```

cgraytracing_amd/csrc/cgrt_hip.hip:

```cpp
#include <hip/hip_runtime.h>

#include <algorithm>
#include <atomic>
#include <chrono>
#include <cmath>
#include <cstdio>
#include <cstdlib>
#include <cstring>
#include <exception>
#include <map>
#include <mutex>
#include <string>
#include <type_traits>
#include <vector>

#include "../../include/cgrt.h"
#include "cgrt_build.h"
#include "cgrt_rng.hpp"
#include "cgrt_types.h"

#include "cgrt_device_math.hpp"
#include "cgrt_grid.hpp"
#include "cgrt_traverse.hpp"
#include "cgrt_bezier.hpp"
// ... 56 lines not shown
    DeviceGuard(const DeviceGuard &) = delete;
    DeviceGuard &operator=(const DeviceGuard &) = delete;
    ~DeviceGuard() {
        if (switched) (void)hipSetDevice(prev);
    }
};
#define ON_DEVICE(dev)          \
    DeviceGuard dev_guard_(dev); \
    if (dev_guard_.err != hipSuccess) return fail(CGRT_ERR_DEVICE, std::string("hipSetDevice: ") + hipGetErrorString(dev_guard_.err))

struct DevBuf {
    void *p = nullptr;
    DevBuf() = default;
    DevBuf(const DevBuf &) = delete;
    DevBuf &operator=(const DevBuf &) = delete;
    ~DevBuf() { if (p) (void)hipFree(p); }
    hipError_t alloc(size_t bytes) { return hipMalloc(&p, bytes ? bytes : 16); }
    void *release() { void *q = p; p = nullptr; return q; }
    template <class T> T *as() { return reinterpret_cast<T *>(p); }
};
class HostStage {
    struct Back { void *host; const void *dev; size_t bytes; };
    std::vector<void *> bufs;
    std::vector<Back> backs;
    int rc_ = CGRT_OK;
    void *alloc(size_t bytes, const void *from, bool zeroed) {
        void *p = nullptr;
        if (rc_) return nullptr;
        hipError_t e = hipMalloc(&p, bytes ? bytes : 16);
        if (e == hipSuccess) bufs.push_back(p);
        if (e == hipSuccess && from) e = hipMemcpy(p, from, bytes, hipMemcpyHostToDevice);
        if (e == hipSuccess && zeroed) e = hipMemset(p, 0, bytes);
        if (e != hipSuccess) rc_ = fail(CGRT_ERR_DEVICE, std::string("host staging: ") + hipGetErrorString(e));
        return rc_ ? nullptr : p;
    }
public:
    HostStage() = default;
    HostStage(const HostStage &) = delete;
    HostStage &operator=(const HostStage &) = delete;
    ~HostStage() { for (void *p : bufs) (void)hipFree(p); }
    int error() const { return rc_; }
    template <class T> T *in(const T *host, size_t bytes) { return host ? static_cast<T *>(alloc(bytes, host, false)) : nullptr; }
    template <class T> T *out(T *host, size_t bytes, bool zeroed = false) { return host ? out_always(host, bytes, zeroed) : nullptr; }
    template <class T> T *out_always(T *host, size_t bytes, bool zeroed = false) {
        T *p = static_cast<T *>(alloc(bytes, nullptr, zeroed));
        if (p && host) backs.push_back({host, p, bytes});
        return p;
    }
    int finish(int rc) {
        if (rc == CGRT_OK) {
            const hipError_t e = hipDeviceSynchronize();
            if (e != hipSuccess) rc = fail(CGRT_ERR_DEVICE, std::string("kernel: ") + hipGetErrorString(e));
        }
        if (rc == CGRT_OK)
            for (const Back &b : backs) HIP_TRY(hipMemcpy(b.host, b.dev, b.bytes, hipMemcpyDeviceToHost));
        return rc;
    }
};

#include "cgrt_tile_order.hpp"

struct cgrt_scene {
    HostScene host;
    bool committed = false;
    int device = -1;
    DeviceScene dev{};
    std::vector<void *> allocs;
    int64_t device_bytes = 0;
    mutable GrowBuf scratch;
    mutable size_t scratch_refused = 0;
    mutable TileOrderState order;
    mutable RelayState relay;
    mutable LensTableState lens;
    size_t mem_total = 0;
    int n_cu = 256;
    hipStream_t aux_stream = nullptr;
    hipEvent_t ev_fork = nullptr, ev_join = nullptr;
    cgrt_build_info build_info{};
    std::vector<TreeRec> tree_recs;
    mutable GrowBuf tri_ids;
    mutable GrowBuf wavefront_work, wavefront_sort;
    mutable WavefrontLast wavefront_last;
    mutable EyeLaunchLog eye_log;
};

template <class T>
static int upload(cgrt_scene *s, const std::vector<T> &v, const T **out, size_t extra = 0) {
    *out = nullptr;
    size_t bytes = (v.size() + extra) * sizeof(T);
    if (bytes == 0) bytes = sizeof(T);
    void *p = nullptr;
    HIP_TRY(hipMalloc(&p, bytes));
    s->allocs.push_back(p);
    s->device_bytes += (int64_t)bytes;
    if (!v.empty()) HIP_TRY(hipMemcpy(p, v.data(), v.size() * sizeof(T), hipMemcpyHostToDevice));
    *out = reinterpret_cast<const T *>(p);
    return CGRT_OK;
}

#include "cgrt_devbuild.hpp"

extern "C" {

int cgrt_version(void) { return CGRT_VERSION; }

int cgrt_look_at(const double eye[3], const double target[3], const double up_hint[3], double fov_x_deg, double focus_distance,
                 double lens_radius, cgrt_posed_camera *out) {
    if (!eye || !target || !up_hint || !out) return fail(CGRT_ERR_INVALID, "cgrt_look_at: null argument");
    if (const char *bad = look_at_camera(eye, target, up_hint, fov_x_deg, focus_distance, lens_radius, out)) return fail(CGRT_ERR_INVALID, bad);
    return CGRT_OK;
}
const char *cgrt_last_error(void) { return g_err.c_str(); }

int cgrt_scene_create(cgrt_scene **out) {
    if (!out) return fail(CGRT_ERR_INVALID, "cgrt_scene_create: null out");
    *out = new (std::nothrow) cgrt_scene();
    if (!*out) return fail(CGRT_ERR_INVALID, "out of memory");
    if (const char *e = std::getenv("CGRT_BUILD")) (*out)->host.build_mode = std::strcmp(e, "device") == 0 ? CGRT_BUILD_DEVICE : CGRT_BUILD_HOST;
    return CGRT_OK;
}

void cgrt_scene_destroy(cgrt_scene *s) {
    if (!s) return;
    if (!s->allocs.empty() || s->scratch.p || s->order.buf.p || s->relay.buf.p || s->lens.buf.p || s->lens.ev || s->tri_ids.p || s->aux_stream || s->order.ev || s->relay.ev) {
        DeviceGuard g(s->device);
        if (g.err == hipSuccess) {
            for (void *p : s->allocs) (void)hipFree(p);
            s->scratch.release();
            s->order.release();
            s->relay.release();
            s->lens.release();
            s->tri_ids.release();
            if (s->ev_fork) (void)hipEventDestroy(s->ev_fork);
            if (s->ev_join) (void)hipEventDestroy(s->ev_join);
            if (s->aux_stream) (void)hipStreamDestroy(s->aux_stream);
        }
    }
    delete s;
}

#define NEED_OPEN(s)                                                          \
    if (!(s)) return fail(CGRT_ERR_INVALID, "null scene");                    \
    if ((s)->committed) return fail(CGRT_ERR_INVALID, "scene already committed")

static int added(cgrt_scene *s, int r) {
    if (r == -2) return fail(CGRT_ERR_IO, s->host.error);
    if (r < 0) return fail(CGRT_ERR_INVALID, s->host.error);
    if ((int)s->host.objs.size() > kMaxObjs) return fail(CGRT_ERR_LIMIT, "more than 2^20 top-level objects");
    return r;
}

int cgrt_scene_set_build(cgrt_scene *s, int mode) {
    NEED_OPEN(s);
    if (mode != CGRT_BUILD_HOST && mode != CGRT_BUILD_DEVICE) return fail(CGRT_ERR_INVALID, "unknown build mode");
    s->host.build_mode = mode;
    return CGRT_OK;
}
int cgrt_scene_build_info(const cgrt_scene *s, cgrt_build_info *out) {
    if (!s || !out) return fail(CGRT_ERR_INVALID, "null argument");
    *out = s->build_info;
    out->mode = s->host.build_mode;
    out->ms_host_build = s->host.host_build_ms;
    return CGRT_OK;
}

int cgrt_scene_add_sphere(cgrt_scene *s, const double c[3], double r, const double sc[3], double refl, double transp) {
// ... 76 lines not shown
            tr.nwide = mr.nwide;
            tr.bmax = tree_bmax(mr.bmax);
            t.dev_nwide = mr.nwide;
            t.wide_stack = mr.stack_need;
            t.dev_balanced = mr.balanced;
            ObjRec &ob = H.objs[(size_t)t.dev_obj];
            for (int k = 0; k < 3; k++) ob.a[k] = mr.centre[k];
            ob.s0 = mr.r2;
            t.dev_cover_at = H.cover.size();
            H.cover.insert(H.cover.end(), mr.cover.begin(), mr.cover.end());
        }
    }
    return CGRT_OK;
}

static int upload_scene(cgrt_scene *s, SceneLayout &L, const CommitKnobs &k, DeviceScene &d, double &ms_device_build) {
    HostScene &H = s->host;
    int rc = CGRT_OK;
    if ((rc = upload(s, L.nodes, &d.nodes))) return rc;
    if ((rc = upload(s, L.tris, &d.tris, L.room_tris))) return rc;
    if ((rc = upload(s, L.texels, &d.texels))) return rc;
    if ((rc = upload(s, L.hcells, &d.hcells, L.room_hcells))) return rc;
    if ((rc = upload(s, L.hcell_y, &d.hcell_y, L.room_hcells))) return rc;
    if ((rc = upload(s, L.otris, &d.otris, L.room_otris))) return rc;
    if ((rc = upload(s, L.tboxes, &d.tboxes))) return rc;
    if ((rc = upload(s, L.wnodes, &d.wnodes, L.room_wnodes))) return rc;
    if (L.n_dev_trees > 0) {
        const auto t_build0 = std::chrono::steady_clock::now();
        if ((rc = device_builds(H, L, d))) return rc;
        ms_device_build = ms_since(t_build0);
    }
    if ((rc = upload(s, H.objs, &d.objs))) return rc;
    if ((rc = upload(s, L.trees, &d.trees))) return rc;
    if ((rc = upload(s, L.texs, &d.texs))) return rc;
    if ((rc = upload(s, H.beziers, &d.beziers))) return rc;
    if ((rc = upload(s, H.bez_slabs, &d.bez_slabs))) return rc;
    if (k.no_bezier_cull) d.bez_slabs = nullptr;
    if ((rc = upload(s, L.hfields, &d.hfields))) return rc;
    if ((rc = upload(s, H.cover, &d.cover))) return rc;
    return CGRT_OK;
}

static void open_light_stream(cgrt_scene *s, AuxPriority priority, DeviceScene &d, bool diffuse) {
    if (!(d.light_ok || diffuse) || s->aux_stream) return;
    int prio_least = 0, prio_greatest = 0;
    (void)hipDeviceGetStreamPriorityRange(&prio_least, &prio_greatest);
    const int prio = priority == AUX_SAME ? 0 : priority == AUX_HIGH ? prio_greatest : prio_least;
    if (hipStreamCreateWithPriority(&s->aux_stream, hipStreamNonBlocking, prio) != hipSuccess ||
        hipEventCreateWithFlags(&s->ev_fork, hipEventDisableTiming) != hipSuccess ||
        hipEventCreateWithFlags(&s->ev_join, hipEventDisableTiming) != hipSuccess) {
        (void)hipGetLastError();
        if (s->ev_fork) (void)hipEventDestroy(s->ev_fork);
        if (s->ev_join) (void)hipEventDestroy(s->ev_join);
        if (s->aux_stream) (void)hipStreamDestroy(s->aux_stream);
        s->ev_fork = s->ev_join = nullptr;
        s->aux_stream = nullptr;
        d.light_ok = 0;
    }
}

int cgrt_scene_commit(cgrt_scene *s, int device) {
    NEED_OPEN(s);
    int ndev = 0;
    HIP_TRY(hipGetDeviceCount(&ndev));
    if (device < 0 || device >= ndev) return fail(CGRT_ERR_DEVICE, "no such HIP device");
    ON_DEVICE(device);
    s->device = device;
    HostScene &H = s->host;
    const auto t_commit0 = std::chrono::steady_clock::now();
    const CommitKnobs knobs = commit_knobs();
    SceneLayout L = scene_layout(H, knobs);
    DeviceScene d{};
    double ms_device_build = 0;
    const size_t cover_host = H.cover.size();
    if (int rc = upload_scene(s, L, knobs, d, ms_device_build)) {
        for (void *p : s->allocs) (void)hipFree(p);
        s->allocs.clear();
        s->device_bytes = 0;
        s->device = -1;
        H.cover.resize(cover_host);
        return rc;
    }
    scene_traits(H, L.trees, knobs, d);
    {
        OrderSpheres &os = s->order.spheres;
        os = OrderSpheres{};
        size_t special = 0;
        for (const ObjRec &o : H.objs) {
            if (o.kind != KIND_SPHERE || (o.refl < kEps && o.transp < kEps)) continue;
            if (special < (size_t)kOrderSpheresMax) {
                for (int k = 0; k < 3; k++) os.s[special][k] = o.a[k];
                os.s[special][3] = std::sqrt(o.s0);
                if (!(o.transp < kEps)) os.transp |= 1u << special;
            }
            special++;
        }
        os.n = (uint32_t)std::min(special, (size_t)kOrderSpheresMax);
        s->order.ok = !d.has_mesh && !d.has_bezier && special >= 1 && special <= (size_t)kOrderSpheresMax;
    }
    open_light_stream(s, knobs.aux_priority, d, s->order.ok && d.all_spheres != 0);
    s->dev = d;
    s->committed = true;
    static std::atomic<uint64_t> commits{0};
    s->order.commit_gen = ++commits;
    s->order.valid = false;
    s->tree_recs = std::move(L.trees);
    size_t fr = 0, tot = 0;
    s->mem_total = hipMemGetInfo(&fr, &tot) == hipSuccess ? tot : ((size_t)32 << 30);
    if (hipDeviceGetAttribute(&s->n_cu, hipDeviceAttributeMultiprocessorCount, device) != hipSuccess || s->n_cu <= 0) {
        (void)hipGetLastError();
        s->n_cu = 256;
    }
    s->build_info.n_device_trees = L.n_dev_trees;
    s->build_info.ms_device_build = ms_device_build;
    s->build_info.ms_commit = ms_since(t_commit0);
    return CGRT_OK;
}

int cgrt_scene_get_stats(const cgrt_scene *s, cgrt_scene_stats *out) {
    if (!s || !out) return fail(CGRT_ERR_INVALID, "null argument");
    std::memset(out, 0, sizeof(*out));
    const HostScene &H = s->host;
    out->n_objects = (int32_t)H.objs.size();
    int64_t bytes = 0;
    for (auto &o : H.objs) {
        if (o.kind == KIND_SPHERE) { out->n_spheres++; bytes += 88; }
        if (o.kind == KIND_PLANE) { out->n_planes++; bytes += 100; }
        if (o.kind == KIND_MESH) out->n_meshes++;
        if (o.kind == KIND_BEZIER) { out->n_beziers++; bytes += 24 * 6 + 100; }
    }
    out->n_textures = (int32_t)H.textures.size();
    out->n_trees = (int32_t)H.trees.size();
    for (auto &t : H.trees) {
        if (t.dev_kind) {
            out->n_triangles += t.dev_ntri;
            out->n_nodes += ref_node_count(t.dev_ntri);
            continue;
        }
        out->n_triangles += (int64_t)t.tris.size();
        out->n_nodes += (int64_t)t.nodes.size();
    }
    bytes += 56 * out->n_nodes + 72 * out->n_triangles;
    for (auto &t : H.textures) bytes += 3 * (int64_t)t.rows * t.cols;
    out->scene_bytes_fp64 = bytes;
    out->device_bytes = s->device_bytes + (int64_t)s->scratch.cap + (int64_t)s->order.buf.cap + (int64_t)s->tri_ids.cap;
    out->committed = s->committed ? 1 : 0;
    return CGRT_OK;
}

int cgrt_scene_tree_sizes(const cgrt_scene *s, int t, int32_t *nnodes, int32_t *nleaftris, int32_t *ntris) {
    if (!s || t < 0 || t >= (int)s->host.trees.size()) return fail(CGRT_ERR_INVALID, "bad tree index");
    const HostTree &T = s->host.trees[t];
    if (nnodes) *nnodes = (int32_t)T.nodes.size();
    if (nleaftris) *nleaftris = (int32_t)T.leaf_ids.size();
    if (ntris) *ntris = T.dev_kind ? (int32_t)T.dev_ntri : (int32_t)(T.tri9.size() / 9);
    return CGRT_OK;
}
int cgrt_scene_bvh_dump(const cgrt_scene *s, int t, int32_t *nnodes, float *box6, int32_t *skip_leaf2) {
    if (!s || t < 0 || t >= (int)s->host.trees.size()) return fail(CGRT_ERR_INVALID, "bad tree index");
    const HostTree &T = s->host.trees[t];
    if (nnodes) *nnodes = T.bvh_nodes;
    for (size_t i = 0; i < T.bvh.size(); i++) {
        if (box6) {
            for (int k = 0; k < 3; k++) {
                box6[6 * i + k] = T.bvh[i].lo[k];
                box6[6 * i + 3 + k] = T.bvh[i].hi[k];
// ... 202 lines not shown
static EyeLaunch light_launch(const DeviceScene &d, bool dof, const EyeKnobs &kn) {
    const bool trees = d.light_trees != 0, hf = trees && d.light_hf_only && !kn.no_hfonly;
    EyeLaunch L;
    L.form = hf ? EyeForm::LightHF : EyeForm::Light;
    L.k = light_flags(trees, dof, hf);
    L.dev = d;
    L.lds = eye_lds(L.k, d);
    return L;
}
static EyeLaunch diffuse_launch(const DeviceScene &d, bool dof) {
    EyeLaunch L;
    L.form = EyeForm::Diffuse;
    L.k = diffuse_flags(dof);
    L.dev = d;
    L.lds = eye_lds(L.k, d);
    return L;
}
static void diffuse_name(const EyeLaunch &L, char *name, size_t cap) {
    std::snprintf(name, cap, "trace_grid_kernel<TREES=0,BEZ=0,DOF=%d,GLASS=0,SPH=1,STATS=0,HPS=0,NT=%d,DIFF=1>", (int)L.k.dof, L.k.nt);
}
static int check_eye(const EyeLaunch &L, int device) {
    const EyeKernels *e = eye_kernels(L.k);
    if (!e) return fail(CGRT_ERR_UNSUPPORTED, std::string(L.what()) + ": no kernel built for this variant");
    return lds_check(reinterpret_cast<const void *>(e->grid), L.lds, device, L.what());
}
static int launch_eye(const EyeLaunch &L, bool sched, const cgrt_scene *s, const GridParams &g, dim3 gd, hipStream_t st, float *rgb,
                      uint32_t *nhit, unsigned long long *cnt, HitpointSink sink = HitpointSink{nullptr, nullptr, 0}) {
    const dim3 block((unsigned)L.k.nt);
    const EyeKernels *e = eye_kernels(L.k);
    if (!e || (sched && !e->sched)) return fail(CGRT_ERR_UNSUPPORTED, std::string(L.what()) + ": no kernel built for this variant");
    const int rc = sched ? launch_checked(e->sched, L.what(), s->device, gd, block, L.lds, st, L.dev, g, rgb, nhit, cnt)
                         : launch_checked(e->grid, L.what(), s->device, gd, block, L.lds, st, L.dev, g, rgb, nhit, cnt, sink);
    if (rc == CGRT_OK) s->eye_log.add(sched ? kEyeSched : kEyeGrid, L.k);
    return rc;
}

static int check_grid_rows(const cgrt_camera *cam, const cgrt_grid *g, bool traced) {
    if (g->width <= 0 || g->height <= 0 || g->rows <= 0) return fail(CGRT_ERR_INVALID, "empty grid");
    if (g->spp <= 0 || (traced && g->spp_total <= 0) || g->sample_offset < 0) return fail(CGRT_ERR_INVALID, "bad sample range");
    if (traced && (g->max_depth < 1 || g->max_depth > kMaxDepth)) return fail(CGRT_ERR_INVALID, "max_depth must be 1..5");
    if (g->stripe_nranks > 1) {
        if (g->stripe_rows <= 0 || g->stripe_rows % kTileH != 0)
            return fail(CGRT_ERR_INVALID, "stripe_rows must be a positive multiple of 8");
        if (g->stripe_rank < 0 || g->stripe_rank >= g->stripe_nranks) return fail(CGRT_ERR_INVALID, "bad stripe_rank");
    } else if (g->row_offset < 0) {
        return fail(CGRT_ERR_INVALID, "bad row_offset");
    }
    if (!(cam->lens_radius >= 0)) return fail(CGRT_ERR_INVALID, "lens_radius must be >= 0");
    if (const char *bad = pose_error(cam, g)) return fail(CGRT_ERR_INVALID, bad);
    return CGRT_OK;
}
static int check_grid(const cgrt_scene *s, const cgrt_camera *cam, const cgrt_grid *g) {
    if (!s || !cam || !g) return fail(CGRT_ERR_INVALID, "null argument");
    if (!s->committed) return fail(CGRT_ERR_INVALID, "scene not committed");
    return check_grid_rows(cam, g, true);
}

static int fit_scratch(const cgrt_scene *s, const FrameInputs &in, FramePlan &p) {
    p = frame_plan(in, fit_heavy_tiles(in, max_heavy_tiles(in), s->scratch_refused));
    while (s->scratch.need(p.scratch.total) != hipSuccess) {
        (void)hipGetLastError();
        if (!s->scratch_refused || p.scratch.total < s->scratch_refused) s->scratch_refused = p.scratch.total;
        if (p.kmax == 0) return fail(CGRT_ERR_DEVICE, "cannot allocate launch scratch (chunk sums / schedule / deferred Hitpoint values)");
        p = frame_plan(in, p.kmax / 2);
    }
    return CGRT_OK;
}

static FrameInputs frame_inputs(const cgrt_scene *s, const cgrt_camera *cam, const cgrt_grid *grid, const EyeLaunch &L, const EyeKnobs &kn) {
    const DeviceScene &d = s->dev;
    FrameInputs in{*grid, *cam, L.form == EyeForm::Sched, L.k.spill, L.k.stats, L.k.glass, L.k.nt, d.has_mesh != 0,
                   d.has_bezier != 0, d.prim_finish != 0, d.light_ok != 0, d.prim_obj, kn, s->mem_total, s->n_cu,
                   L.k.nt == 64 ? kBezWaves : (L.k.trees ? kSchedTreeWaves : 4)};
    in.image = L.form == EyeForm::Image;
    in.sph = L.k.sph;
    in.pair = L.k.pair;
    in.order_ok = s->order.ok;
    in.aux_stream = s->aux_stream != nullptr;
    in.all_spheres = d.all_spheres != 0;
    in.n_objs = d.n_objs;
    in.n_lds = d.n_lds;
    in.all_special = order_all_special(s->order.spheres, *cam);
    in.posed = L.k.pose;
    if (in.posed) in.posed_cam = *reinterpret_cast<const cgrt_posed_camera *>(cam);
    return in;
}

static int probe_and_plan(const cgrt_scene *s, const EyeLaunch &L, const EyeKnobs &kn, const FramePlan &p, const GridParams &g,
                          unsigned char *scratch, hipStream_t st, float *rgb, uint32_t *nhit, unsigned long long *cnt) {
    const ScratchLayout &at = p.scratch;
    unsigned char *light = at.light.in<unsigned char>(scratch);
    if (light)
        hipLaunchKernelGGL(classify_kernel, dim3((unsigned)((p.n_wt + 255) / 256)), dim3(256), 0, st, s->dev, g, light, (int)p.n_wt);
    GridParams gp = g;
    gp.spp = gp.chunks = gp.chunk_spp = 1;
    gp.probe = 1;
    gp.cost = at.cost.in<uint32_t>(scratch);
    gp.light = light;
    int rc = launch_eye(L, false, s, gp, dim3((unsigned)p.tile_blocks), st, nullptr, nullptr, nullptr);
    if (rc) return rc;
    if (light) {
        GridParams gl = g;
        gl.light = light;
        gl.light_mode = 1;
        gl.xcd_tiles = 0;
        HIP_TRY(hipEventRecord(s->ev_fork, st));
        HIP_TRY(hipStreamWaitEvent(s->aux_stream, s->ev_fork, 0));
        if ((rc = launch_eye(light_launch(s->dev, L.k.dof, kn), false, s, gl,
                             dim3((unsigned)tile_grid_blocks(g.W, g.rows, false)), s->aux_stream, rgb, nhit, cnt)))
            return rc;
        HIP_TRY(hipEventRecord(s->ev_join, s->aux_stream));
    }
    const int tw = L.k.nt == 64 ? 1 : kTileW / kWaveTileW, th = L.k.nt == 64 ? 1 : kTileH / kWaveTileH;
    hipLaunchKernelGGL(plan_kernel, dim3(1), dim3(1024), 0, st, gp.cost, light, (int)p.n_wt, (unsigned)p.kmax, p.plan_div,
                       at.plan.in<uint32_t>(scratch), at.order.in<uint32_t>(scratch), at.hidx.in<int32_t>(scratch),
                       at.border.in<uint32_t>(scratch), p.wtiles_x, p.wtiles_y, tw, th);
    return CGRT_OK;
}

static EyeLaunch start_twin(EyeLaunch L) {
    L.k.start = true;
    return L;
}
static EyeLaunch table_twin(EyeLaunch L) {
    L.k.ltab = true;
    return L;
}
static int relay_cost_start(const cgrt_scene *s, const EyeLaunch &L, const FramePlan &p, GridParams &g, hipStream_t st) {
    CostStart c;
    if (int rc = cost_start_begin(s->order, p.relay, g, st, c)) return rc;
    if (!c.wcost) return CGRT_OK;
    if (!c.have_cost) {
        GridParams gp = g;
        gp.probe = 2;
        gp.cost = c.wcost;
        gp.spp = gp.chunk_spp = p.relay.probe_spp;
        gp.sample_offset = 0;
        gp.accumulate = 0;
        gp.tile_order = kOrderFull;
        gp.relay = nullptr;
        gp.relay_k = 0;
        gp.relay_start_at = gp.relay_boost_at = 0;
        gp.lens_table = nullptr;
        gp.lens_table_cap = gp.lens_table_spp = 0;
        if (int rc = launch_eye(start_twin(L), false, s, gp, dim3((unsigned)p.grid_dim), st, nullptr, nullptr, nullptr)) return rc;
    }
    return cost_start_rank(s->order, p, c, g, st);
}

static int primary_walk(const cgrt_scene *s, const EyeLaunch &L, const GridParams &g, hipStream_t st, unsigned long long *cnt) {
    PrimWalkArgs pw;
    pw.len = const_cast<double *>(g.prim_len);
    pw.tri = const_cast<int32_t *>(g.prim_tri);
    pw.obj = s->dev.prim_obj;
    pw.tree = s->host.objs[(size_t)s->dev.prim_obj].tree;
    pw.finish = g.prim_done;
    pw.pad_ = 0;
    pw.counters = cnt;
    const size_t staged = (size_t)(pw.finish ? s->dev.n_objs : pw.obj + 1);
    const int rc = launch_checked(L.k.dof ? &primary_walk_kernel<true> : &primary_walk_kernel<false>, "primary_walk_kernel", s->device,
                                  dim3((unsigned)s->n_cu * 4), dim3(kThreads), primary_walk_lds(staged), st, s->dev, g, pw);
    if (rc == CGRT_OK) {
        EyeFlags walk{};
        walk.dof = L.k.dof;
        s->eye_log.add(kEyePrimaryWalk, walk);
    }
    return rc;
}

static int write_timeline(const char *file, const DevBuf &tl, size_t n_blocks, const GridParams &g, int nt, hipStream_t st) {
    std::vector<unsigned long long> rec(n_blocks * 4);
    HIP_TRY(hipStreamSynchronize(st));
    HIP_TRY(hipMemcpy(rec.data(), tl.p, rec.size() * 8, hipMemcpyDeviceToHost));
    if (FILE *f = std::fopen(file, "wb")) {
        const unsigned long long form = (unsigned long long)g.relay_k | (unsigned long long)g.relay_extent << 8 | (unsigned long long)g.relay_order << 9;
        const unsigned long long head[4] = {n_blocks, (unsigned long long)nt, (unsigned long long)g.chunks,
                                            g.relay_k > 1 ? (form << 32 | (unsigned long long)g.relay_cap) : (unsigned long long)g.xcd_tiles};
        std::fwrite(head, 8, 4, f);
        std::fwrite(rec.data(), 8, rec.size(), f);
        std::fclose(f);
    }
    return CGRT_OK;
}
static int dump_plan(const FramePlan &p, const GridParams &g, hipStream_t st) {
    uint32_t pl[8] = {0};
    HIP_TRY(hipStreamSynchronize(st));
    HIP_TRY(hipMemcpy(pl, g.plan, sizeof(pl), hipMemcpyDeviceToHost));
    std::fprintf(stderr, "cgrt plan: wave tiles %zu, heavy %u (capacity %zu), cost threshold %u, tile-queue entries %u, items per tile %d, prim walk %s\n",
                 p.n_wt, pl[0], p.kmax, pl[1], pl[3], g.items_per_tile, g.prim_len ? "on" : "off");
    return CGRT_OK;
}

extern "C" {

int cgrt_trace_grid_variant(const cgrt_scene *s, const cgrt_camera *cam, const cgrt_grid *grid, char *name, size_t cap) {
    int rc = check_grid(s, cam, grid);
    if (rc) return rc;
    if (!name || cap == 0) return fail(CGRT_ERR_INVALID, "null name buffer");
    ON_DEVICE(s->device);
    const EyeLaunch L = eye_launch(s, cam, grid, eye_knobs(), (grid->flags & CGRT_GRID_HITPOINTS) != 0);
    const EyeFlags &k = L.k;
    const bool sched = L.form == EyeForm::Sched;
    if (!eye_kernels(k)) return fail(CGRT_ERR_UNSUPPORTED, std::string(L.what()) + ": no kernel built for this variant");
    std::snprintf(name, cap, "trace_grid_%skernel<TREES=%d,BEZ=%d,DOF=%d,GLASS=%d,SPH=%d,STATS=%d,%s%sNT=%d%s%s>", sched ? "sched_" : "",
                  (int)k.trees, (int)k.bez, (int)k.dof, (int)k.glass, (int)k.sph, (int)k.stats,
                  sched ? "" : (k.hps ? "HPS=1," : "HPS=0,"), k.pair ? "PAIR=1," : "", k.nt, k.spill ? ",SPILL=1" : "", k.pose ? ",POSE=1" : "");
    return CGRT_OK;
}

int cgrt_trace_grid(const cgrt_scene *s, const cgrt_camera *cam, const cgrt_grid *grid, float *rgb, uint32_t *nhit,
                    uint64_t *counters, void *stream) {
    int rc = check_grid(s, cam, grid);
    if (rc) return rc;
    if (!rgb) return fail(CGRT_ERR_INVALID, "null rgb");
    hipStream_t st = reinterpret_cast<hipStream_t>(stream);
    auto *cnt = reinterpret_cast<unsigned long long *>(counters);
    ON_DEVICE(s->device);
    const EyeKnobs kn = eye_knobs();
    s->eye_log.clear();
    const EyeLaunch L0 = eye_launch(s, cam, grid, kn, false);
    if (L0.k.pose && (rc = check_eye(L0, s->device))) return rc;
    const FrameInputs in = frame_inputs(s, cam, grid, L0, kn);
    FramePlan p;
    if ((rc = fit_scratch(s, in, p))) return rc;
    GridParams g = frame_params(in, p);
    unsigned char *scratch = reinterpret_cast<unsigned char *>(s->scratch.p);
    if (p.heavy_blocks > 0 && (rc = probe_and_plan(s, L0, kn, p, g, scratch, st, rgb, nhit, cnt))) return rc;
    p.scratch.place(g, scratch, nhit != nullptr);
    size_t n_blocks = (size_t)p.heavy_blocks + p.grid_dim;
    TileOrderGuard guard(s->order, s->relay);
    LensTableGuard lens(s->lens, st);
    bool tabled = false;
    EyeLaunch L = L0;
    if (p.order.on) {
        const Capturing capturing = stream_capturing(st);
        if ((rc = order_tiles(s->order, s->dev, p, g, kn.no_order_reuse, capturing, st))) return rc;
        const bool beside_probe = p.relay.relays() && p.relay.start == kRelayStartCost && cost_probe_due(s->order, p.relay, g);
        if (p.order.lens_table_cap > 0 && (tabled = lens_table_prepare(s->lens, s->order, p, g, kn.no_order_reuse, beside_probe, capturing, st, s->aux_stream)))
            L = table_twin(L0);
        if (p.relay.relays() && relay_prepare(s->relay, p.relay, g, capturing, st)) {
            guard.relayed = &p.relay;
            if (p.relay.start == kRelayStartCost && (rc = relay_cost_start(s, L0, p, g, st))) return rc;
            n_blocks = p.relay.grid(p.grid_dim, g.relay_boost_at != 0);
        }
        if ((rc = lens_table_join(s->lens, st))) return rc;
    }
    DevBuf timeline;
    if (kn.timeline_file) {
        HIP_TRY(timeline.alloc(n_blocks * 32));
        HIP_TRY(hipMemsetAsync(timeline.p, 0, n_blocks * 32, st));
        g.timeline = timeline.as<unsigned long long>();
    }
    if (p.heavy_blocks > 0) {
        if (L.k.pose) hipLaunchKernelGGL(pixel_const_kernel<true>, dim3((unsigned)p.kmax), dim3(64), 0, st, g);
        else hipLaunchKernelGGL(pixel_const_kernel<false>, dim3((unsigned)p.kmax), dim3(64), 0, st, g);
        if (g.prim_len && (rc = primary_walk(s, L, g, st, cnt))) return rc;
        if ((rc = launch_eye(L, true, s, g, dim3((unsigned)n_blocks), st, rgb, nhit, cnt))) return rc;
    } else if (p.order.class3 == TileOrderPlan::SecondLaunch) {
        const EyeLaunch DL = diffuse_launch(s->dev, L.k.dof);
        if ((rc = check_eye(DL, s->device))) return rc;
        GridParams gd = g;
        g.tile_order = kOrderFull;
        gd.tile_order = kOrderDiffuse;
        HIP_TRY(hipEventRecord(s->ev_fork, st));
        if ((rc = launch_eye(L, false, s, g, dim3((unsigned)n_blocks), st, rgb, nhit, cnt))) return rc;
        HIP_TRY(hipStreamWaitEvent(s->aux_stream, s->ev_fork, 0));
        if ((rc = launch_eye(DL, false, s, gd, dim3((unsigned)n_blocks), s->aux_stream, rgb, nhit, cnt))) return rc;
        HIP_TRY(hipEventRecord(s->ev_join, s->aux_stream));
    } else {
        if (p.order.class3 == TileOrderPlan::InKernel) g.tile_order = kOrderAllDiffuse;
        if ((rc = launch_eye(g.relay_start_at ? start_twin(L) : L, false, s, g, dim3((unsigned)n_blocks), st, rgb, nhit, cnt))) return rc;
    }
    if (p.chunks > 1)
        hipLaunchKernelGGL(finalize_chunks_kernel, dim3((unsigned)(((size_t)g.rows * g.W + 255) / 256)), dim3(256), 0, st, g, rgb, nhit);
    if (p.heavy_blocks > 0) hipLaunchKernelGGL(deferred_sum_kernel, dim3((unsigned)p.kmax), dim3(64), 0, st, g, rgb, nhit);
    if (g.light || p.order.class3 == TileOrderPlan::SecondLaunch) HIP_TRY(hipStreamWaitEvent(st, s->ev_join, 0));
    const hipError_t launch_err = hipGetLastError();
    if (g.timeline && launch_err == hipSuccess && (rc = write_timeline(kn.timeline_file, timeline, n_blocks, g, L.k.nt, st))) return rc;
    if (launch_err != hipSuccess) return fail(CGRT_ERR_DEVICE, std::string("kernel launch: ") + hipGetErrorString(launch_err));
    if ((rc = guard.commit(g, st))) return rc;
    if ((rc = lens.commit(tabled))) return rc;
    return kn.plan_dump && g.plan && !g.tile_order ? dump_plan(p, g, st) : CGRT_OK;
}

#define NEED_COMMITTED(s, args_ok)                                           \
    if (!(s) || !(args_ok)) return fail(CGRT_ERR_INVALID, "null argument"); \
    if (!(s)->committed) return fail(CGRT_ERR_INVALID, "scene not committed")

int cgrt_scene_last_tile_order(const cgrt_scene *s, uint32_t *plan5, uint32_t *list, uint8_t *cls, int64_t cap, int64_t *n_tiles) {
    NEED_COMMITTED(s, n_tiles);
    ON_DEVICE(s->device);
    return last_tile_order(s->order, plan5, list, cls, cap, n_tiles);
}
int cgrt_scene_last_sphere_masks(const cgrt_scene *s, uint32_t *masks, int64_t cap, int64_t *n_wave_tiles) {
    NEED_COMMITTED(s, n_wave_tiles);
    ON_DEVICE(s->device);
    return last_sphere_masks(s->order, masks, cap, n_wave_tiles);
}
int cgrt_scene_last_sure_tiles(const cgrt_scene *s, uint8_t *sure, int64_t cap, int64_t *n_wave_tiles) {
    NEED_COMMITTED(s, n_wave_tiles);
    ON_DEVICE(s->device);
    return last_sure_tiles(s->order, sure, cap, n_wave_tiles);
}
int cgrt_scene_last_tile_order_reused(const cgrt_scene *s, int32_t *reused) {
    NEED_COMMITTED(s, reused);
    *reused = s->order.reused ? 1 : 0;
    return CGRT_OK;
}
int cgrt_scene_last_diffuse_tiles(const cgrt_scene *s, int64_t *n_tiles) {
    NEED_COMMITTED(s, n_tiles);
    ON_DEVICE(s->device);
    return last_class3_tiles(s->order, TileOrderPlan::SecondLaunch, n_tiles);
}
int cgrt_scene_last_inkernel_diffuse_tiles(const cgrt_scene *s, int64_t *n_tiles) {
    NEED_COMMITTED(s, n_tiles);
    ON_DEVICE(s->device);
    return last_class3_tiles(s->order, TileOrderPlan::InKernel, n_tiles);
}
int cgrt_scene_last_lens_stage(const cgrt_scene *s, int64_t *lds_tiles, int64_t *area_tiles) {
    NEED_COMMITTED(s, lds_tiles && area_tiles);
    ON_DEVICE(s->device);
    return last_lens_stage(s->order, lds_tiles, area_tiles);
}
int cgrt_scene_last_lens_table(const cgrt_scene *s, int64_t *entries, int64_t *capacity, int32_t *reused) {
    NEED_COMMITTED(s, entries && capacity && reused);
    ON_DEVICE(s->device);
    return last_lens_table(s->order, s->lens, entries, capacity, reused);
}
int cgrt_scene_inside_spheres(const cgrt_scene *s, int32_t *index, uint32_t *mask, double *rin2, int32_t cap, int32_t *n) {
    NEED_COMMITTED(s, n && (cap <= 0 || (index && mask && rin2)));
    const InsideTrait &t = s->dev.inside;
    *n = t.n;
    for (int k = 0; k < t.n && k < cap; k++) index[k] = t.idx[k], mask[k] = t.mask[k], rin2[k] = t.rin2[k];
    return CGRT_OK;
}
int cgrt_scene_last_sample_relay(const cgrt_scene *s, int64_t *tiles, int32_t *chunks, int64_t *parked_values) {
    NEED_COMMITTED(s, tiles && chunks && parked_values);
    ON_DEVICE(s->device);
    return last_sample_relay(s->order, s->relay, tiles, chunks, parked_values);
}
int cgrt_scene_last_relay_form(const cgrt_scene *s, int32_t *mirror, int32_t *order) {
    NEED_COMMITTED(s, mirror && order);
    last_relay_form(s->order, s->relay, mirror, order);
    return CGRT_OK;
}

int cgrt_scene_last_relay_start(const cgrt_scene *s, uint32_t *start, int64_t start_cap, uint32_t *wcost, int64_t cost_cap, int64_t *t,
                                int64_t *n_wave_tiles, int32_t *reused) {
    NEED_COMMITTED(s, t && n_wave_tiles && reused);
    ON_DEVICE(s->device);
    return last_relay_start(s->order, s->relay, start, start_cap, wcost, cost_cap, t, n_wave_tiles, reused);
}

int cgrt_scene_last_relay_boost(const cgrt_scene *s, int64_t *promoted, int32_t *k_boost, int64_t *boost_cap, uint64_t *cost_sum, int32_t *num,
                                int32_t *den, int32_t *wg_slots, uint32_t *bslot, int64_t slot_cap) {
    NEED_COMMITTED(s, promoted && k_boost && boost_cap && cost_sum && num && den && wg_slots);
    ON_DEVICE(s->device);
    return last_relay_boost(s->order, s->relay, promoted, k_boost, boost_cap, cost_sum, num, den, wg_slots, bslot, slot_cap);
}

int cgrt_scene_last_eye_launches(const cgrt_scene *s, int32_t *rows, int64_t cap, int64_t *n) {
    NEED_COMMITTED(s, n && (cap <= 0 || rows));
    const EyeLaunchLog &log = s->eye_log;
    *n = log.n;
    for (int i = 0; i < log.n && i < cap; i++) log.row(i, rows + (size_t)i * kEyeLogCols);
    return log.overflow ? fail(CGRT_ERR_LIMIT, "eye pass: more launches than the handle's record holds") : CGRT_OK;
}

int cgrt_trace_grid_diffuse_variant(const cgrt_scene *s, const cgrt_camera *cam, const cgrt_grid *grid, char *name, size_t cap) {
    int rc = check_grid(s, cam, grid);
    if (rc) return rc;
    if (!name || cap == 0) return fail(CGRT_ERR_INVALID, "null name buffer");
    ON_DEVICE(s->device);
    const EyeKnobs kn = eye_knobs();
    const EyeLaunch L = eye_launch(s, cam, grid, kn, false);
    name[0] = 0;
    if (frame_plan(frame_inputs(s, cam, grid, L, kn), 0).order.class3 == TileOrderPlan::SecondLaunch)
        diffuse_name(diffuse_launch(s->dev, L.k.dof), name, cap);
    return CGRT_OK;
}

}


__global__ void unpermute_stripes_kernel(const float *__restrict__ shares, int n_present, int nshares, int row_floats, int S,
                                         int rows_local, float *__restrict__ frame) {
    const int h = blockIdx.y, x = blockIdx.x * blockDim.x + threadIdx.x;
    if (x >= row_floats) return;
    const int stripe = h / S, share = stripe % nshares, j = (stripe / nshares) * S + h % S;
    float v = 0.f;
    if (share < n_present && j < rows_local) v = shares[((size_t)share * rows_local + (size_t)j) * row_floats + x];
    frame[(size_t)h * row_floats + x] = v;
}

static int capture_finish(const char *what, DevBuf &b_rec, DevBuf &b_cnt, uint64_t cap, double **d_rec_out, uint64_t *count) {
    *count = 0;
    hipError_t e = hipGetLastError();
    if (e == hipSuccess) e = hipDeviceSynchronize();
    if (e != hipSuccess) return fail(CGRT_ERR_DEVICE, std::string(what) + hipGetErrorString(e));
    unsigned long long n = 0;
    if (hipMemcpy(&n, b_cnt.p, sizeof(n), hipMemcpyDeviceToHost) != hipSuccess) return fail(CGRT_ERR_DEVICE, "hitpoint count copy");
    *count = n;
    if (cap && d_rec_out) *d_rec_out = reinterpret_cast<double *>(b_rec.release());
    return CGRT_OK;
}
static int hitpoints_to_host(int rc, double *d_rec, uint64_t n, double *hp10, uint64_t cap, uint64_t *count) {
    if (rc == CGRT_OK) {
        *count = n;
        const uint64_t m = n < cap ? n : cap;
        if (m && hipMemcpy(hp10, d_rec, (size_t)m * 10 * sizeof(double), hipMemcpyDeviceToHost) != hipSuccess)
            rc = fail(CGRT_ERR_DEVICE, "hitpoint copy");
    }
    if (d_rec) (void)hipFree(d_rec);
    return rc;
}

static int hitpoints_device(const cgrt_scene *s, const cgrt_camera *cam, const cgrt_grid *grid, uint64_t cap,
                            double **d_rec_out, uint64_t *count) {
// ... 226 lines not shown
```

cgraytracing_amd/csrc/cgrt_scene_walk.hpp:

```cpp
#ifndef CGRT_SCENE_WALK_HPP
#define CGRT_SCENE_WALK_HPP
#include "cgrt_bezier.hpp"
#include "cgrt_traverse.hpp"
#include "cgrt_wg_lds.h"

__device__ __forceinline__ bool texture_color(const TexRec &t, const uint8_t *__restrict__ texels, V3 point, V3 &out) {
    V3 d = point - ld3(t.p);
    const V3 n = ld3(t.n);
    d = d - n * dot(d, n);
    const double te = 1e-2;
    const int rows = t.rows, cols = t.cols;
    int r, c;
    if (d.x < te && d.x > -te) {
        if (!(0 < d.y && d.y < t.lenx && 0 < d.z && d.z < t.leny)) return false;
        r = (int)floor(d.y / t.lenx * rows);
        c = (int)floor(d.z / t.leny * cols);
    } else if (d.y < te && d.y > -te) {
        if (!(0 < d.x && d.x < t.lenx && 0 < d.z && d.z < t.leny)) return false;
        c = (int)floor(d.x / t.lenx * cols);
        r = (int)floor(d.z / t.leny * rows);
    } else if (d.z < te && d.z > -te) {
        if (!(0 < d.x && d.x < t.lenx && 0 < d.y && d.y < t.leny)) return false;
        c = (int)floor(d.x / t.lenx * cols);
        r = rows - 1 - (int)floor(d.y / t.leny * rows);
// ... 194 lines not shown
    p.aux.lnodes = l.has.nodes ? reinterpret_cast<NodeRec *>(lds_raw + l.nodes) : nullptr;
    p.aux.wstack = l.has.wstack ? reinterpret_cast<uint2 *>(lds_raw + l.wstack) : nullptr;
    return p;
}
template <int NT>
__device__ __forceinline__ void wg_stage16(void *dst, const void *src, int n16) {
    const uint4 *s = reinterpret_cast<const uint4 *>(src);
    uint4 *d = reinterpret_cast<uint4 *>(dst);
    for (int k = threadIdx.x; k < n16; k += NT) d[k] = s[k];
}

template <bool STATS, bool HFONLY = false>
__device__ __forceinline__ TreeHit tree_hit(const DeviceScene &sc, const LdsAux &aux, int tr, bool opaque, double bound,
                                            bool on, V3 o, V3 d, V3 inv, uint32_t &n_node, uint32_t &n_tri) {
    const TreeRec T = load_uniform(sc.trees + tr);
    TreeHit none;
    none.len = kInf;
    none.tri = -1;
    none.counter = 0;
    UTILP(1, on);
    if (!on) return none;
    if (HFONLY || (opaque && T.hfield >= 0)) {
        const HFieldRec H = load_uniform(sc.hfields + T.hfield);
        return hfield_intersect<STATS>(H, sc.hcells + H.cell_begin, sc.hcell_y + H.cell_begin, o, d, inv, bound, n_node, n_tri);
    }
    const bool cached = aux.lnodes != nullptr && tr == sc.cached_tree;
    const Ray32 r32 = make_ray32(o, inv, T.bmax);
    const int oct = (T.noct == 8 && opaque) ? ((d.x < 0 ? 1 : 0) | (d.y < 0 ? 2 : 0) | (d.z < 0 ? 4 : 0)) : 0;
    const NodeRec *nodes = sc.nodes + T.node_begin + (size_t)oct * (size_t)T.nnodes;
    const TriRec *tris = sc.tris + T.tri_begin;
    if (opaque) {
        if (T.tri_level) {
            if (T.nwide == 0) return none;
            return tree_intersect_wide<STATS>(sc.wnodes + T.wnode_begin, sc.otris + T.otri_begin, o, d, r32, bound, n_node, n_tri,
                                              aux.wstack);
        }
        if (cached) return tree_intersect<STATS, true>(aux.lnodes, tris, T.nnodes, o, d, r32, bound, n_node, n_tri);
        return tree_intersect<STATS, true>(nodes, tris, T.nnodes, o, d, r32, bound, n_node, n_tri);
    }
    const NodeRec *tb = sc.tboxes + T.tbox_begin;
    if (cached) return tree_intersect_lq<STATS>(aux.lnodes, tris, T.nnodes, o, d, r32, n_node, n_tri, tb);
    return tree_intersect_lq<STATS>(nodes, tris, T.nnodes, o, d, r32, n_node, n_tri, tb);
}

template <bool TREES, bool BEZ, bool SPH, bool STATS, bool SPILL = false, bool PRE = false, bool HFONLY = false, bool NRM = true,
          bool PAIR = false, bool MASKED = false>
__device__ __forceinline__ SceneHit intersect_scene(const ObjRec *__restrict__ objs, int n_lds, int n_objs, const DeviceScene &sc,
                                                    V3 o, V3 d, RayKey &rk, bool on, const LdsAux &aux,
                                                    uint32_t &n_node, uint32_t &n_tri, bool masked = false, uint32_t mask = 0u) {
    SceneHit best;
    best.t = kInf;
    best.id = -1;
    best.n = mk(0, 0, 0);
    int nsrc = 0;
    if (SPH) {
        static_assert(!PAIR || (SPH && !SPILL), "PAIR: the LDS-resident sphere loop");
        static_assert(!MASKED || (SPH && !SPILL && !PAIR && !NRM), "MASKED: the terminal-diffuse body's sphere loop");
        if (MASKED && masked) {
            for (uint32_t m = mask; m != 0u; m &= m - 1u) {
                const int i = __builtin_ctz(m);
                const double len = sphere_len(objs[i], o, d);
                if (len < best.t) {
                    best.t = len;
                    best.id = i;
                }
            }
            return best;
        }
        int i_single = 0;
        if (PAIR) {
            for (int k = 0; k < kInsideMax && k < sc.inside.n; k++) {
                const bool in = starts_inside(o, ld3(objs[sc.inside.idx[k]].a), sc.inside.rin2[k]);
                if (__ballot(on && !in) != 0ull) continue;
                for (uint32_t m = sc.inside.mask[k]; m != 0u; m &= m - 1u) {
                    const int i = __builtin_ctz(m);
                    const double len = sphere_len(objs[i], o, d);
                    if (len < best.t) {
                        best.t = len;
                        best.id = i;
                    }
                }
                return best;
            }
            for (int i = 0; i + 1 < n_lds; i += 2) {
                double lenA, lenB;
                const ObjRec &A = objs[i], &B = objs[i + 1];
                sphere_len_pair(ld3(A.a), A.s0, ld3(B.a), B.s0, o, d, lenA, lenB);
                if (lenA < best.t) {
                    best.t = lenA;
                    best.id = i;
                }
                if (lenB < best.t) {
                    best.t = lenB;
                    best.id = i + 1;
                }
            }
            i_single = n_lds & ~1;
        }
        for (int i = i_single; i < n_lds; i++) {
            const double len = sphere_len(objs[i], o, d);
            if (len < best.t) {
                best.t = len;
                best.id = i;
            }
        }
        for (int i = n_lds; SPILL && i < n_objs; i++) {
            const ObjHead h = load_uniform(reinterpret_cast<const ObjHead *>(sc.objs + i));
            const double len = sphere_len(mk(h.a[0], h.a[1], h.a[2]), h.s0, o, d);
            if (len < best.t) {
                best.t = len;
                best.id = i;
            }
        }
        if (NRM && best.id >= 0) best.n = normalized((o + d * best.t) - load_centre<SPILL>(objs, n_lds, sc.objs, best.id));
        return best;
    }
    V3 inv = mk(0, 0, 0);
    bool inv_ready = false;
    constexpr bool FRONT = HFONLY || BEZ;
    bool run_unsure = false, run_skip = false;
    int run_begin = 0, run_end = 0, i_first = 0;
    if (!SPH && sc.prun_end > 0 && (FRONT || sc.prun_begin == 0)) {
        run_begin = FRONT ? sc.prun_begin : 0;
        run_end = sc.prun_end;
        const PlaneRunHit ph = plane_run(objs, run_begin, run_end, o, d);
        run_unsure = ph.unsure;
        if (!ph.unsure && ph.id >= 0 && ph.len > 0) {
            if (ph.len < best.t) {
                best.t = ph.len;
                best.id = ph.id;
                best.n = ld3(objs[ph.id].b);
                nsrc = 1;
            }
        }
        run_skip = __ballot(run_unsure) == 0ull;
        if (run_skip && run_begin == 0) i_first = run_end;
    }
    for (int i = i_first; i < (SPILL ? n_objs : n_lds); i++) {
        const ObjRec *obp = objs + i;
        if (SPILL && i >= n_lds) {
            if ((threadIdx.x & 63) < 8)
                reinterpret_cast<uint4 *>(aux.spill)[threadIdx.x & 63] = reinterpret_cast<const uint4 *>(sc.objs + i)[threadIdx.x & 63];
            __builtin_amdgcn_fence(__ATOMIC_ACQ_REL, "wavefront");
            __builtin_amdgcn_wave_barrier();
            obp = aux.spill;
        }
        const ObjRec &ob = *obp;
        if (FRONT && run_skip && i >= run_begin && i < run_end) continue;
        const bool planes_one_by_one = !((!FRONT || i >= run_begin) && i < run_end) || run_unsure;
        const int kind = __builtin_amdgcn_readfirstlane(ob.kind);
        if (kind == KIND_SPHERE) {
            const double len = sphere_len(ob, o, d);
            if (len < best.t) {
                best.t = len;
                best.id = i;
                nsrc = 0;
            }
        } else if (kind == KIND_PLANE) {
            const V3 pn = ld3(ob.b);
            const double len_plane = plane_len(ob, pn, o, d);
            double len = len_plane;
            const bool ph = len > 0;
            V3 nrm = pn;
            if (TREES) {
                const int tr = __builtin_amdgcn_readfirstlane(ob.tree);
                const bool want = on && ph;
                if (tr >= 0 && __ballot(want) != 0ull) {
                    if (!inv_ready) {
                        inv = mk(1.0 / d.x, 1.0 / d.y, 1.0 / d.z);
                        inv_ready = true;
                    }
                    const bool opaque = __builtin_amdgcn_readfirstlane((int)(ob.transp < kEps)) != 0;
                    const TreeHit h = tree_hit<STATS, HFONLY>(sc, aux, tr, opaque, fmin(len, best.t), want, o, d, inv, n_node, n_tri);
                    if (want && h.counter > 0 && h.len < len && h.len > 0) {
                        len = h.len;
                        nrm = tree_normal(sc.tris + load_uniform(&sc.trees[tr].tri_begin), h, d);
                    }
                }
            }
            if (planes_one_by_one && ph && (len < best.t || (FRONT && i < run_begin && len == best.t && best.id >= run_begin))) {
// ... 66 lines not shown
```

cgraytracing_amd/csrc/cgrt_types.h:

```cpp
#ifndef CGRT_TYPES_H
#define CGRT_TYPES_H
#include <stddef.h>
#include <stdint.h>

#include "cgrt_inside_sphere.h"

namespace cgrt {

static constexpr double kEps = 1e-4;
static constexpr double kInf = 1e10;
static constexpr int kMinKd = 10;
static constexpr double kBoxPad = 1.001e-4;
static constexpr int kMaxDepth = 5;

enum ObjKind : int32_t { KIND_SPHERE = 0, KIND_PLANE = 1, KIND_MESH = 2, KIND_BEZIER = 3 };

struct ObjRec {
    double a[3];
    double b[3];
    double s0;
    double col[3];
    double refl, transp;
    int32_t kind;
    int32_t tree;
    int32_t tex;
    int32_t aux;
    int32_t axis;
    int32_t pad1, pad2, pad3;
};
static_assert(sizeof(ObjRec) == 128, "ObjRec layout");

struct NodeRec {
    float lo[3];
    float hi[3];
    int32_t skip;
    int32_t leaf;
};
static_assert(sizeof(NodeRec) == 32, "NodeRec layout");

struct TriRec {
    double pa[3];
    double e1[3];
    double e2[3];
};

struct OTriRec {
    TriRec t;
    int32_t k;
    int32_t leaf;
};
static_assert(sizeof(OTriRec) == 80, "OTriRec layout");

struct WideNodeRec {
    float lox[4], loy[4], loz[4], hix[4], hiy[4], hiz[4];
    int32_t ref[4];
    int32_t pad[4];
};
static_assert(sizeof(WideNodeRec) == 128, "WideNodeRec layout");
static constexpr int32_t kWideNone = INT32_MIN;
static constexpr int kWideLdsDepth = 16;
static constexpr int kWideStack = 64;

struct TreeRec {
    int64_t node_begin;
    int64_t tri_begin;
    int64_t otri_begin;
    int32_t nnodes;
    int32_t ntris;
    int32_t hfield;
    int32_t noct;
    int32_t tri_level;
    float bmax;
    int64_t tbox_begin;
    int64_t wnode_begin;
    int32_t nwide;
    int32_t pad2;
};

struct HCellRec {
    TriRec t[2];
    int32_t k[2];
    int32_t leaf[2];
};
static_assert(sizeof(HCellRec) == 160, "HCellRec layout");
struct HFieldRec {
    int64_t cell_begin;
    int32_t nx, nz;
    double x0, z0;
    double hx, hz;
    double ylo, yhi;
    double ihx, ihz;
};
struct HCellY {
    float lo, hi;
};

struct TexRec {
    int64_t texel_begin;
    int32_t rows, cols;
    double n[3];
    double p[3];
    double lenx, leny;
    int32_t isbump;
    int32_t pad;
};

struct BezierRec {
    double cp[6][3];
    int32_t ncp;
    int32_t pad;
    double box[6];
};

struct BezSlabRec {
    double ylo, yhi, r2, pad;
};
static constexpr int kBezSlabs = 64;

static constexpr int kLdsObjsMax = 768;
static constexpr size_t kLdsBytes = (size_t)160 << 10;
static constexpr int kMaxObjs = 1 << 20;
static constexpr int kNodeCache = 256;

struct DeviceScene {
    const ObjRec *objs;
    const NodeRec *nodes;
    const TriRec *tris;
    const TreeRec *trees;
    const TexRec *texs;
    const uint8_t *texels;
    const BezierRec *beziers;
    const HFieldRec *hfields;
    const HCellRec *hcells;
    const HCellY *hcell_y;
    const OTriRec *otris;
    const NodeRec *tboxes;
    const WideNodeRec *wnodes;
    const BezSlabRec *bez_slabs;
    const double *cover;
    int32_t n_objs, n_trees, n_texs, n_beziers;
    int32_t n_lds;
    int32_t prim_obj;
    int32_t has_mesh;
    int32_t has_bezier;
    int32_t all_spheres;
    int32_t has_glass;
    int32_t cached_tree;
    int32_t cached_nodes;
    int32_t has_wide;
    int32_t light_trees;
    int32_t light_ok;
    int32_t n_cover;
    int32_t prim_finish;
    int32_t prun_begin, prun_end;
    int32_t single_ray;
    int32_t light_hf_only;
    InsideTrait inside;
};

}
#endif
```

include/cgrt.h:

```cpp
#ifndef CGRT_H
#define CGRT_H

#include <stddef.h>
#include <stdint.h>

#ifdef __cplusplus
extern "C" {
#endif

#define CGRT_VERSION 112

enum {
    CGRT_OK = 0,
    CGRT_ERR_INVALID = -1,
    CGRT_ERR_IO = -2,
    CGRT_ERR_DEVICE = -3,
    CGRT_ERR_UNSUPPORTED = -4,
    CGRT_ERR_LIMIT = -5
};

typedef struct cgrt_scene cgrt_scene;

typedef struct cgrt_camera {
    double cam[3];
    double half_width;
    double focus_plane;
    double lens_radius;
} cgrt_camera;

typedef struct cgrt_posed_camera {
    cgrt_camera base;
    double origin[3];
    double right[3], up[3], forward[3];
} cgrt_posed_camera;

int cgrt_look_at(const double eye[3], const double target[3], const double up_hint[3], double fov_x_deg, double focus_distance,
                 double lens_radius, cgrt_posed_camera *out);

typedef struct cgrt_grid {
    int32_t width, height;
    int32_t rows;
    int32_t row_offset;
    int32_t stripe_rows;
    int32_t stripe_rank;
    int32_t stripe_nranks;
    int32_t spp;
    int32_t sample_offset;
    int32_t spp_total;
    int32_t max_depth;
    int32_t flags;
    uint64_t seed;
} cgrt_grid;

enum {
    CGRT_GRID_STATS = 1,
    CGRT_GRID_ACCUMULATE = 2,
    CGRT_GRID_NO_REORDER = 8,
    CGRT_GRID_FORCE_REORDER = 16,
    CGRT_GRID_NO_TILE_ORDER = 64,
    CGRT_GRID_DIFFUSE_TILES = 128,
    CGRT_GRID_NO_SPHERE_PAIRS = 256,
    CGRT_GRID_NO_SPHERE_MASKS = 512,
    CGRT_GRID_SAMPLE_RELAY = 1024,
    CGRT_GRID_NO_SAMPLE_RELAY = 2048,
    CGRT_GRID_SAMPLE_RELAY_4 = 4096,
    CGRT_GRID_RELAY_MIRROR = 8192,
    CGRT_GRID_RELAY_NO_MIRROR = 16384,
    CGRT_GRID_RELAY_CHUNKS_FIRST = 32768,
    CGRT_GRID_RELAY_MIRROR_FIRST = 65536,
    CGRT_GRID_RELAY_INTERLEAVED = 98304,
    CGRT_GRID_RELAY_ORDER_MASK = 98304,
    CGRT_GRID_RELAY_COST_START = 524288,
    CGRT_GRID_NO_RELAY_COST_START = 1048576,
    CGRT_GRID_RELAY_BOOST = 2097152,
    CGRT_GRID_NO_RELAY_BOOST = 4194304,
    CGRT_GRID_NO_LENS_STAGE = 131072,
    CGRT_GRID_NO_LENS_TABLE = 8388608,
    CGRT_GRID_LENS_TABLE = 16777216,
    CGRT_GRID_NO_SURE_TILES = 262144,
    CGRT_GRID_NO_INSIDE_TRIPS = 33554432,
    CGRT_GRID_POSED = 67108864,
    CGRT_GRID_HITPOINTS = 32,
    CGRT_GRID_SPLIT_SAMPLES = 4
};

enum {
    CGRT_CNT_RAYS = 0,
    CGRT_CNT_HITPOINTS = 1,
    CGRT_CNT_WAVE_ITERS = 2,
    CGRT_CNT_NODE_TESTS = 3,
    CGRT_CNT_TRI_TESTS = 4,
    CGRT_NCOUNTERS = 8
};

typedef struct cgrt_scene_stats {
    int32_t n_objects, n_spheres, n_planes, n_meshes, n_beziers, n_textures, n_trees, committed;
    int64_t n_triangles;
    int64_t n_nodes;
    int64_t device_bytes;
    int64_t scene_bytes_fp64;
} cgrt_scene_stats;

int cgrt_version(void);
const char *cgrt_last_error(void);

int cgrt_scene_create(cgrt_scene **out);
void cgrt_scene_destroy(cgrt_scene *s);

enum { CGRT_BUILD_HOST = 0, CGRT_BUILD_DEVICE = 1 };
int cgrt_scene_set_build(cgrt_scene *s, int mode);

typedef struct cgrt_build_info {
    int32_t mode;
    int32_t n_device_trees;
    double ms_host_build;
    double ms_device_build;
    double ms_commit;
} cgrt_build_info;
int cgrt_scene_build_info(const cgrt_scene *s, cgrt_build_info *out);

int cgrt_scene_add_sphere(cgrt_scene *s, const double c[3], double r, const double sc[3], double refl, double transp);

int cgrt_scene_add_texture(cgrt_scene *s, const uint8_t *rgb, int rows, int cols, const double n[3],
                           const double p[3], double lx, double ly, int isbump);

int cgrt_scene_add_plane(cgrt_scene *s, const double p[3], const double n[3], const double sc[3], double refl,
                         double transp, int tex_id);

int cgrt_scene_add_mesh_file(cgrt_scene *s, const char *filename, double a, const double b[3], const double sc[3],
                             double refl, double transp, int typeofdata);
int cgrt_scene_add_mesh_triangles(cgrt_scene *s, const double *tri9, int ntri, const double sc[3], double refl,
                                  double transp, int typeofdata);

int cgrt_scene_add_bezier(cgrt_scene *s, const double *cp3, int ncp, const double pos[3], const double sc[3],
                          double refl, double transp);

int cgrt_scene_commit(cgrt_scene *s, int device);
int cgrt_scene_get_stats(const cgrt_scene *s, cgrt_scene_stats *out);

int cgrt_scene_tree_sizes(const cgrt_scene *s, int t, int32_t *nnodes, int32_t *nleaftris, int32_t *ntris);
int cgrt_scene_tree_dump(const cgrt_scene *s, int t, int32_t *node_lr_size, int32_t *leaf_ids, double *bbox,
                         double *tri9);

int cgrt_scene_bvh_dump(const cgrt_scene *s, int tree, int32_t *nnodes, float *box6, int32_t *skip_leaf2);
int cgrt_scene_bvh_order(const cgrt_scene *s, int tree, int32_t *tri_level, int32_t *order);
int cgrt_scene_wide_dump(const cgrt_scene *s, int tree, int32_t *nwide, int32_t *stack_need, float *box24, int32_t *ref4);

int cgrt_trace_grid(const cgrt_scene *s, const cgrt_camera *cam, const cgrt_grid *grid, float *rgb,
                    uint32_t *nhit, uint64_t *counters, void *stream);

typedef struct cgrt_rays {
    int64_t n;
    const double *org3;
    const double *dir3;
    const uint64_t *keys;
    int64_t first_index;
    uint64_t seed;
    int32_t max_depth;
    int32_t flags;
} cgrt_rays;
enum {
    CGRT_RAYS_STATS = 1,
    CGRT_RAYS_NO_SIGN_PASS = 2,
// ... 154 lines not shown
int cgrt_ppm_session_add_photons(cgrt_ppm_session *p, int64_t count);
typedef struct cgrt_photon_rays {
    int64_t n;
    const double *org3;
    const double *dir3;
    const double *flux3;
    const uint64_t *keys;
    const uint32_t *draws;
} cgrt_photon_rays;
int cgrt_ppm_session_add_photon_rays(cgrt_ppm_session *p, const cgrt_photon_rays *pr);
int cgrt_photon_emit(const cgrt_photons *ph, int64_t first, int64_t count, double *org3, double *dir3, double *flux3,
                     uint64_t *keys, uint32_t *draws, void *stream);
int cgrt_photon_emit_host(const cgrt_photons *ph, int64_t first, int64_t count, double *org3, double *dir3, double *flux3,
                          uint64_t *keys, uint32_t *draws);

int cgrt_ppm_session_image(const cgrt_ppm_session *p, double *image, uint8_t *rgb8);
int cgrt_ppm_session_image_device(const cgrt_ppm_session *p, double *image, uint8_t *rgb8, void *stream);
int cgrt_ppm_session_hitpoints(const cgrt_ppm_session *p, double *hp16, uint64_t cap, uint64_t *count);
typedef struct cgrt_ppm_session_info {
    int64_t photons_done;
    uint64_t hp_count, n_events, n_pairs, n_batch_halvings;
    int64_t device_bytes;
    double ms_eye, ms_table;
    double ms_photons;
    double ms_last_add, ms_last_image;
} cgrt_ppm_session_info;
int cgrt_ppm_session_get_info(const cgrt_ppm_session *p, cgrt_ppm_session_info *out);

typedef struct cgrt_sppm_session cgrt_sppm_session;
int cgrt_sppm_session_create(const cgrt_scene *s, int32_t width, int32_t rows, int32_t spp, int32_t photon_depth,
                             const cgrt_photons *ph, int32_t flags, cgrt_sppm_session **out);
void cgrt_sppm_session_destroy(cgrt_sppm_session *p);
int cgrt_sppm_session_pass_grid(cgrt_sppm_session *p, const cgrt_camera *cam, const cgrt_grid *grid, int64_t nphotons);
int cgrt_sppm_session_pass_rays(cgrt_sppm_session *p, const cgrt_rays *rays, const int64_t *pixel, int64_t nphotons);
int cgrt_sppm_session_image(const cgrt_sppm_session *p, double *image, uint8_t *rgb8);
int cgrt_sppm_session_image_device(const cgrt_sppm_session *p, double *image, uint8_t *rgb8, void *stream);
int cgrt_sppm_session_pixels(const cgrt_sppm_session *p, double *px8);
int cgrt_sppm_session_last_hitpoints(const cgrt_sppm_session *p, double *hp16, uint64_t cap, uint64_t *count);
typedef struct cgrt_sppm_session_info {
    int64_t passes, photons_done;
    uint64_t hp_count;
    uint64_t n_events, n_pairs, n_batch_halvings;
    int64_t device_bytes;
    double ms_eye, ms_table, ms_photons, ms_update;
} cgrt_sppm_session_info;
int cgrt_sppm_session_get_info(const cgrt_sppm_session *p, cgrt_sppm_session_info *out);
int cgrt_sppm_update_host(double N, double R2, const double *tau3, double M, const double *phi3, double alpha, double *out5);
int cgrt_sppm_check_host(int32_t width, int32_t rows, int32_t spp, int32_t photon_depth, const cgrt_photons *ph, int32_t flags,
                         const cgrt_grid *grid);

int cgrt_tonemap_rgb8(int device, const double *image, int width, int height, uint8_t *rgb8);

int cgrt_write_png(const char *path, int width, int height, const uint8_t *rgb8);

int cgrt_photon_events(const cgrt_scene *s, const cgrt_photons *ph, int max_depth, int64_t first, int32_t count,
                       double *events9, uint8_t *valid);

int cgrt_photon_ray_events(const cgrt_scene *s, const cgrt_photon_rays *pr, uint64_t seed, int64_t first_index, int max_depth,
                           double *events9, uint8_t *valid);

int cgrt_intersect_rays(const cgrt_scene *s, int obj, const double *org3, const double *dir3, const uint64_t *keys,
                        int n, int32_t *hit, double *len, double *normal3);

int cgrt_surface_colors(const cgrt_scene *s, int obj, const double *points3, int n, double *colors3);

int cgrt_trace_grid_variant(const cgrt_scene *s, const cgrt_camera *cam, const cgrt_grid *grid, char *name, size_t cap);

int cgrt_scene_last_tile_order(const cgrt_scene *s, uint32_t *plan5, uint32_t *list, uint8_t *cls, int64_t cap, int64_t *n_tiles);

int cgrt_scene_last_sphere_masks(const cgrt_scene *s, uint32_t *masks, int64_t cap, int64_t *n_wave_tiles);
int cgrt_scene_last_sure_tiles(const cgrt_scene *s, uint8_t *sure, int64_t cap, int64_t *n_wave_tiles);
int cgrt_scene_last_tile_order_reused(const cgrt_scene *s, int32_t *reused);

int cgrt_trace_grid_diffuse_variant(const cgrt_scene *s, const cgrt_camera *cam, const cgrt_grid *grid, char *name, size_t cap);
int cgrt_scene_last_diffuse_tiles(const cgrt_scene *s, int64_t *n_tiles);
int cgrt_scene_last_inkernel_diffuse_tiles(const cgrt_scene *s, int64_t *n_tiles);
int cgrt_scene_last_sample_relay(const cgrt_scene *s, int64_t *tiles, int32_t *chunks, int64_t *parked_values);
int cgrt_scene_last_relay_form(const cgrt_scene *s, int32_t *mirror, int32_t *order);
int cgrt_scene_last_relay_start(const cgrt_scene *s, uint32_t *start, int64_t start_cap, uint32_t *wcost, int64_t cost_cap, int64_t *t,
                                int64_t *n_wave_tiles, int32_t *reused);
int cgrt_scene_last_lens_stage(const cgrt_scene *s, int64_t *lds_tiles, int64_t *area_tiles);
int cgrt_scene_last_lens_table(const cgrt_scene *s, int64_t *entries, int64_t *capacity, int32_t *reused);
int cgrt_scene_inside_spheres(const cgrt_scene *s, int32_t *index, uint32_t *mask, double *rin2, int32_t cap, int32_t *n);
int cgrt_scene_last_eye_launches(const cgrt_scene *s, int32_t *rows, int64_t cap, int64_t *n);

int cgrt_relay_start_host(int32_t k, int32_t chunk_spp, int32_t spp, int64_t cap, int32_t extent, int64_t n01, int64_t n012, int64_t n_tiles,
                          const uint32_t *list, const uint32_t *wcost, int32_t width, int32_t rows, uint32_t *start, int64_t start_cap,
                          int64_t *t);

int cgrt_scene_last_relay_boost(const cgrt_scene *s, int64_t *promoted, int32_t *k_boost, int64_t *boost_cap, uint64_t *cost_sum,
                                int32_t *num, int32_t *den, int32_t *wg_slots, uint32_t *bslot, int64_t slot_cap);
int cgrt_relay_boost_host(int32_t k, int32_t chunk_spp, int32_t spp, int64_t cap, int32_t extent, int64_t n01, int64_t n012, int64_t n_tiles,
                          const uint32_t *list, const uint32_t *wcost, int32_t width, int32_t rows, int32_t k_boost, int32_t boost_chunk_spp,
                          int64_t boost_cap, int32_t num, int32_t den, int32_t wg_slots, uint32_t *start, int64_t start_cap, uint32_t *bslot,
                          int64_t slot_cap, int64_t *t, int64_t *promoted, uint64_t *cost_sum);

int cgrt_lens_samples(uint64_t seed, const int64_t *pixel, const int32_t *sample, int n, double radius, double *out3);

enum { CGRT_PROBE_SQRT = 0, CGRT_PROBE_NORMALIZED = 1, CGRT_PROBE_SPHERE_LEN = 2, CGRT_PROBE_SPHERE_LEN_PAIR = 4  };
int cgrt_math_probe(int device, int op, const double *in, int64_t n, double *out);
enum { CGRT_PROBE_INSIDE_LOOP = 5 };
int cgrt_inside_probe(const cgrt_scene *s, int op, const double *rays, int64_t n, double *out);

#ifdef __cplusplus
}
#endif
#endif
```

Before: 120,500.

## Cull spheres nested inside opaque diffuse occluders from terminal-diffuse eye launches

Adds a commit-time analysis that finds spheres fully enclosed by an opaque, non-reflective sphere far from any specular object, and marks them unreachable. When the camera lens lies outside every such occluder, the terminal-diffuse PAIR body runs on a compacted object list (or a masked walk) that omits the hidden spheres, with the sphere masks, sure-tile indices and inside-trip tables remapped to match. This is meant to cut per-ray sphere intersection tests and LDS footprint. It adds an extra template variant, index remapping, and a conservative geometric validity check that can disable the path.

```diff
diff --git a/cgraytracing_amd/_capi.py b/cgraytracing_amd/_capi.py
--- a/cgraytracing_amd/_capi.py
+++ b/cgraytracing_amd/_capi.py
@@ -52,6 +52,7 @@
 GRID_RELAY_COST_START, GRID_NO_RELAY_COST_START, GRID_RELAY_BOOST, GRID_NO_RELAY_BOOST = 524288, 1048576, 2097152, 4194304
 GRID_NO_LENS_TABLE, GRID_LENS_TABLE = 8388608, 16777216
 GRID_NO_INSIDE_TRIPS = 33554432
+GRID_NO_UNREACHABLE = 134217728
 GRID_POSED = 67108864
 
 
@@ -273,6 +274,8 @@
                                       C.c_void_p, C.c_void_p, C.c_void_p]),
     "cgrt_math_probe": (C.c_int, [C.c_int, C.c_int, C.c_void_p, C.c_int64, C.c_void_p]),
     "cgrt_scene_inside_spheres": (C.c_int, [C.c_void_p, C.c_void_p, C.c_void_p, C.c_void_p, C.c_int32, C.POINTER(C.c_int32)]),
+    "cgrt_scene_unreachable_spheres": (C.c_int, [C.c_void_p, C.POINTER(C.c_int32), C.POINTER(C.c_uint32), C.c_void_p, C.c_int32,
+                                                  C.POINTER(C.c_int32), C.POINTER(C.c_uint32)]),
     "cgrt_inside_probe": (C.c_int, [C.c_void_p, C.c_int, C.c_void_p, C.c_int64, C.c_void_p]),
 }
 
diff --git a/cgraytracing_amd/csrc/cgrt_build.cpp b/cgraytracing_amd/csrc/cgrt_build.cpp
--- a/cgraytracing_amd/csrc/cgrt_build.cpp
+++ b/cgraytracing_amd/csrc/cgrt_build.cpp
@@ -1035,6 +1035,19 @@
         }
         d.inside = inside_trait(balls.data(), transp.data(), d.n_objs, true);
     }
-}
-
-}
+    d.reach = 0;
+}
+
+UnreachTrait scene_unreachable(const HostScene &H, const DeviceScene &d) {
+    if (!d.all_spheres || d.n_objs != d.n_lds || d.n_objs > kUnreachSpheresMax) return UnreachTrait{};
+    std::vector<InsideBall> balls;
+    std::vector<double> refl, transp;
+    for (const ObjRec &o : H.objs) {
+        balls.push_back(InsideBall{{o.a[0], o.a[1], o.a[2]}, o.s0});
+        refl.push_back(o.refl);
+        transp.push_back(o.transp);
+    }
+    return unreach_trait(balls.data(), refl.data(), transp.data(), d.n_objs);
+}
+
+}
diff --git a/cgraytracing_amd/csrc/cgrt_build.h b/cgraytracing_amd/csrc/cgrt_build.h
--- a/cgraytracing_amd/csrc/cgrt_build.h
+++ b/cgraytracing_amd/csrc/cgrt_build.h
@@ -5,6 +5,7 @@
 #include <vector>
 
 #include "cgrt_types.h"
+#include "cgrt_unreachable_sphere.h"
 
 namespace cgrt {
 
@@ -102,6 +103,7 @@
 SceneLayout scene_layout(const HostScene &H, const CommitKnobs &k);
 
 void scene_traits(const HostScene &H, const std::vector<TreeRec> &trees, const CommitKnobs &k, DeviceScene &d);
+UnreachTrait scene_unreachable(const HostScene &H, const DeviceScene &d);
 
 }
 #endif
diff --git a/cgraytracing_amd/csrc/cgrt_eye.hpp b/cgraytracing_amd/csrc/cgrt_eye.hpp
--- a/cgraytracing_amd/csrc/cgrt_eye.hpp
+++ b/cgraytracing_amd/csrc/cgrt_eye.hpp
@@ -81,7 +81,8 @@
 }
 
 template <bool TREES, bool BEZ, bool DOF, bool GLASS, bool SPH, bool STATS, bool HPS, int NT, bool HEAVY, bool SPILL = false, bool HFONLY = false,
-          bool DIFF = false, bool PAIR = false, bool PARK = false, bool LSTAGE = false, bool COST = false, bool LTAB = false, bool POSE = false>
+          bool DIFF = false, bool PAIR = false, bool PARK = false, bool LSTAGE = false, bool COST = false, bool LTAB = false, bool POSE = false,
+          bool REACH = false>
 __device__ __forceinline__ void trace_grid_body(const DeviceScene &sc, const GridParams &g, float *__restrict__ rgb,
                                                 uint32_t *__restrict__ nhit_out, unsigned long long *__restrict__ counters,
                                                 const HitpointSink &hps, int tile_block, int tile_grid, const RelayWg rw = RelayWg{},
@@ -93,6 +94,7 @@
     static_assert(!PAIR || (SPH && GLASS && !HPS && !HEAVY && !STATS && !SPILL), "PAIR: the glass sphere variants of the tile order");
     static_assert(!LSTAGE || (DIFF && DOF && !PAIR), "LSTAGE: the thin-lens terminal-diffuse body inside a PAIR launch");
     static_assert(!COST || PAIR, "COST: the PAIR variants with a start table");
+    static_assert(!REACH || (DIFF && !PAIR), "REACH: the terminal-diffuse body inside a PAIR launch");
     static_assert(!POSE || (!DIFF && !PAIR && !LSTAGE && !LTAB), "POSE: no body of the tile order, whose tests stand in the built-in frame");
     static_assert(!LSTAGE || lens_batch_lds(NT) <= (size_t)kLdsLevels * pending_level_bytes(NT), "the lens batches fit the PAIR launch's pending-ray levels");
     const long long tl_t0 = g.timeline ? wall_clock64() : 0;
@@ -193,12 +195,15 @@
     uint32_t smask = 0u;
     if (masked) {
         smask = load_uniform(g.wmask + __builtin_amdgcn_readfirstlane(have_tile ? wy * wtiles_x + wx : 0));
+        if (REACH && sc.reach != 0u) smask = kReachWalk ? (smask & sc.reach) : unreach_compact(smask, sc.reach);
         if (sc.n_lds < 32) smask &= (1u << sc.n_lds) - 1u;
     }
     uint32_t sure = (uint32_t)kSureNone;
     if (DIFF && g.wsure != nullptr && have_tile) {
         const uint32_t wt = (uint32_t)__builtin_amdgcn_readfirstlane(wy * wtiles_x + wx);
         sure = (load_uniform(reinterpret_cast<const uint32_t *>(g.wsure) + (wt >> 2)) >> ((wt & 3u) * 8u)) & 0xffu;
+        if (REACH && !kReachWalk && sc.reach != 0u)
+            sure = (sure < 32u && ((sc.reach >> sure) & 1u)) ? (uint32_t)unreach_compact_index((int)sure, sc.reach) : (uint32_t)kSureNone;
         if (sure >= (uint32_t)sc.n_lds) sure = (uint32_t)kSureNone;
     }
     uint64_t k_smp = 0;
@@ -760,7 +765,7 @@
     __shared__ unsigned long long wg_cnt[CGRT_NCOUNTERS];
     unsigned long long *wc = wg_counters_begin(wg_cnt, counters);
     if (PAIR && g.tile_order == kOrderAllDiffuse && entry >= load_uniform(g.plan + 3))
-        trace_grid_body<false, false, DOF, false, true, false, false, NT, false, false, false, true, false, false, DOF>(sc, g, rgb, nhit_out, wc, hps, tile_block, tile_grid);
+        trace_grid_body<false, false, DOF, false, true, false, false, NT, false, false, false, true, false, false, DOF, false, false, false, true>(sc, g, rgb, nhit_out, wc, hps, tile_block, tile_grid);
     else if (LTAB && g.lens_table != nullptr && entry < (unsigned)g.lens_table_cap && entry < load_uniform(g.plan + 3)) {
         const uint64_t *lens_row = g.lens_table + (size_t)entry * (size_t)g.lens_table_spp * NT;
         if (rw.chunk > 0)
@@ -1358,6 +1363,7 @@
     aux.lnodes = nullptr;
     uint32_t nn = 0, nt = 0;
     sc.inside = InsideTrait{};
+    sc.reach = 0u;
     const SceneHit a = intersect_scene<false, false, true, false, false, false, false, false, true>(sc.objs, sc.n_lds, sc.n_objs, sc, o, d, rk, true, aux, nn, nt);
     sc.inside = guarded;
     const SceneHit b = intersect_scene<false, false, true, false, false, false, false, false, true>(sc.objs, sc.n_lds, sc.n_objs, sc, o, d, rk, true, aux, nn, nt);
diff --git a/cgraytracing_amd/csrc/cgrt_frame.h b/cgraytracing_amd/csrc/cgrt_frame.h
--- a/cgraytracing_amd/csrc/cgrt_frame.h
+++ b/cgraytracing_amd/csrc/cgrt_frame.h
@@ -11,6 +11,7 @@
 #include "../../include/cgrt.h"
 #include "cgrt_lens_stage.h"
 #include "cgrt_relay.h"
+#include "cgrt_unreachable_sphere.h"
 
 struct GridParams {
     int32_t W, H, rows, row_offset, stripe_rows, stripe_rank, stripe_nranks;
@@ -275,6 +276,7 @@
     long long lens_table_bytes = 0;
     bool lens_table_bytes_set = false;
     bool no_inside_trips = false;
+    bool no_unreachable = false;
     const char *timeline_file = nullptr;
 };
 inline const char *env_str(const char *name) { const char *e = std::getenv(name); return e ? e : ""; }
@@ -370,6 +372,12 @@
             if (!v.empty() && !k.no_inside_trips && v != "on" && v != "1")
                 std::fprintf(stderr, "cgrt: CGRT_INSIDE_TRIPS=%s is neither off nor on: the default is used\n", v.c_str());
         }
+        {
+            const std::string v(env_str("CGRT_UNREACHABLE"));
+            k.no_unreachable = v == "off" || v == "0";
+            if (!v.empty() && !k.no_unreachable && v != "on" && v != "1")
+                std::fprintf(stderr, "cgrt: CGRT_UNREACHABLE=%s is neither off nor on: the default is used\n", v.c_str());
+        }
         return k;
     }();
     EyeKnobs k = once;
@@ -401,6 +409,7 @@
     bool all_special = false;
     bool posed = false;
     cgrt_posed_camera posed_cam{};
+    UnreachTrait unreach{};
 };
 
 struct ScratchLayout {
@@ -543,6 +552,7 @@
     ScratchLayout scratch;
     TileOrderPlan order;
     RelayPlan relay;
+    uint32_t reach = 0;
 };
 
 inline FramePlan frame_plan(const FrameInputs &in, size_t kmax) {
@@ -589,6 +599,9 @@
         o.lens_table_bytes = lens_table_bytes(o.lens_table_cap, gr.spp, kThreads);
         o.lens_table_always = o.lens_table_cap > 0 && (lens_table > 0 || kLensTableAlways);
     }
+    if (in.pair && !in.posed && in.unreach.n == in.n_lds && in.n_objs == in.n_lds && !(gr.flags & CGRT_GRID_NO_UNREACHABLE) && !kn.no_unreachable &&
+        unreach_launch_ok(in.unreach, in.cam.cam, in.cam.lens_radius))
+        p.reach = in.unreach.reach;
     p.wtiles_x = (gr.width + kWaveTileW - 1) / kWaveTileW;
     p.wtiles_y = (gr.rows + kWaveTileH - 1) / kWaveTileH;
     p.n_wt = (size_t)p.wtiles_x * p.wtiles_y;
diff --git a/cgraytracing_amd/csrc/cgrt_hip.hip b/cgraytracing_amd/csrc/cgrt_hip.hip
--- a/cgraytracing_amd/csrc/cgrt_hip.hip
+++ b/cgraytracing_amd/csrc/cgrt_hip.hip
@@ -162,6 +162,9 @@
     mutable GrowBuf wavefront_work, wavefront_sort;
     mutable WavefrontLast wavefront_last;
     mutable EyeLaunchLog eye_log;
+    UnreachTrait unreach{};
+    mutable uint32_t last_reach = 0;
+    const ObjRec *reach_objs = nullptr;
 };
 
 template <class T>
@@ -404,6 +407,17 @@
         return rc;
     }
     scene_traits(H, L.trees, knobs, d);
+    s->unreach = scene_unreachable(H, d);
+    s->reach_objs = nullptr;
+    if (unreach_drops(s->unreach)) {
+        std::vector<ObjRec> kept;
+        for (int j = 0; j < s->unreach.n; j++)
+            if ((s->unreach.reach >> j) & 1u) kept.push_back(H.objs[(size_t)j]);
+        if (upload(s, kept, &s->reach_objs) != CGRT_OK) {
+            (void)hipGetLastError();
+            s->reach_objs = nullptr;
+        }
+    }
     {
         OrderSpheres &os = s->order.spheres;
         os = OrderSpheres{};
@@ -772,6 +786,7 @@
     in.n_lds = d.n_lds;
     in.all_special = order_all_special(s->order.spheres, *cam);
     in.posed = L.k.pose;
+    in.unreach = s->unreach;
     if (in.posed) in.posed_cam = *reinterpret_cast<const cgrt_posed_camera *>(cam);
     return in;
 }
@@ -908,11 +923,25 @@
     ON_DEVICE(s->device);
     const EyeKnobs kn = eye_knobs();
     s->eye_log.clear();
-    const EyeLaunch L0 = eye_launch(s, cam, grid, kn, false);
+    EyeLaunch L0 = eye_launch(s, cam, grid, kn, false);
     if (L0.k.pose && (rc = check_eye(L0, s->device))) return rc;
     const FrameInputs in = frame_inputs(s, cam, grid, L0, kn);
     FramePlan p;
+    s->last_reach = 0;
     if ((rc = fit_scratch(s, in, p))) return rc;
+    if (p.reach != 0u && (kReachWalk || s->reach_objs)) {
+        L0.dev.reach = s->last_reach = p.reach;
+        for (int k = 0; k < L0.dev.inside.n; k++) L0.dev.inside.mask[k] &= p.reach;
+        if (!kReachWalk) {
+            L0.dev.objs = s->reach_objs;
+            L0.dev.n_objs = L0.dev.n_lds = __builtin_popcount(p.reach);
+            for (int k = 0; k < L0.dev.inside.n; k++) {
+                L0.dev.inside.mask[k] = unreach_compact(L0.dev.inside.mask[k], p.reach);
+                L0.dev.inside.idx[k] = unreach_compact_index(L0.dev.inside.idx[k], p.reach);
+            }
+            L0.lds = eye_lds(L0.k, L0.dev) + (L0.form == EyeForm::Image || L0.form == EyeForm::Sched ? (size_t)kn.lds_pad : 0);
+        }
+    }
     GridParams g = frame_params(in, p);
     unsigned char *scratch = reinterpret_cast<unsigned char *>(s->scratch.p);
     if (p.heavy_blocks > 0 && (rc = probe_and_plan(s, L0, kn, p, g, scratch, st, rgb, nhit, cnt))) return rc;
@@ -1024,6 +1053,17 @@
     for (int k = 0; k < t.n && k < cap; k++) index[k] = t.idx[k], mask[k] = t.mask[k], rin2[k] = t.rin2[k];
     return CGRT_OK;
 }
+int cgrt_scene_unreachable_spheres(const cgrt_scene *s, int32_t *n, uint32_t *reach, int32_t *occluder, int32_t cap, int32_t *n_occ,
+                                   uint32_t *last) {
+    NEED_COMMITTED(s, n && reach && n_occ && last && (cap <= 0 || occluder));
+    const UnreachTrait &t = s->unreach;
+    *n = t.n;
+    *reach = t.reach;
+    *n_occ = t.n_occ;
+    for (int k = 0; k < t.n_occ && k < cap; k++) occluder[k] = t.occ[k].idx;
+    *last = s->last_reach;
+    return CGRT_OK;
+}
 int cgrt_scene_last_sample_relay(const cgrt_scene *s, int64_t *tiles, int32_t *chunks, int64_t *parked_values) {
     NEED_COMMITTED(s, tiles && chunks && parked_values);
     ON_DEVICE(s->device);
diff --git a/cgraytracing_amd/csrc/cgrt_scene_walk.hpp b/cgraytracing_amd/csrc/cgrt_scene_walk.hpp
--- a/cgraytracing_amd/csrc/cgrt_scene_walk.hpp
+++ b/cgraytracing_amd/csrc/cgrt_scene_walk.hpp
@@ -300,20 +300,50 @@
                 }
                 return best;
             }
-            for (int i = 0; i + 1 < n_lds; i += 2) {
-                double lenA, lenB;
-                const ObjRec &A = objs[i], &B = objs[i + 1];
-                sphere_len_pair(ld3(A.a), A.s0, ld3(B.a), B.s0, o, d, lenA, lenB);
-                if (lenA < best.t) {
-                    best.t = lenA;
-                    best.id = i;
-                }
-                if (lenB < best.t) {
-                    best.t = lenB;
-                    best.id = i + 1;
-                }
-            }
-            i_single = n_lds & ~1;
+            if (kReachWalk && sc.reach != 0u) {
+                uint32_t m = sc.reach;
+                while ((m & (m - 1u)) != 0u) {
+                    const int ia = __builtin_ctz(m);
+                    m &= m - 1u;
+                    const int ib = __builtin_ctz(m);
+                    m &= m - 1u;
+                    double lenA, lenB;
+                    const ObjRec &A = objs[ia], &B = objs[ib];
+                    sphere_len_pair(ld3(A.a), A.s0, ld3(B.a), B.s0, o, d, lenA, lenB);
+                    if (lenA < best.t) {
+                        best.t = lenA;
+                        best.id = ia;
+                    }
+                    if (lenB < best.t) {
+                        best.t = lenB;
+                        best.id = ib;
+                    }
+                }
+                if (m != 0u) {
+                    const int i = __builtin_ctz(m);
+                    const double len = sphere_len(objs[i], o, d);
+                    if (len < best.t) {
+                        best.t = len;
+                        best.id = i;
+                    }
+                }
+                i_single = n_lds;
+            } else {
+                for (int i = 0; i + 1 < n_lds; i += 2) {
+                    double lenA, lenB;
+                    const ObjRec &A = objs[i], &B = objs[i + 1];
+                    sphere_len_pair(ld3(A.a), A.s0, ld3(B.a), B.s0, o, d, lenA, lenB);
+                    if (lenA < best.t) {
+                        best.t = lenA;
+                        best.id = i;
+                    }
+                    if (lenB < best.t) {
+                        best.t = lenB;
+                        best.id = i + 1;
+                    }
+                }
+                i_single = n_lds & ~1;
+            }
         }
         for (int i = i_single; i < n_lds; i++) {
             const double len = sphere_len(objs[i], o, d);
diff --git a/cgraytracing_amd/csrc/cgrt_types.h b/cgraytracing_amd/csrc/cgrt_types.h
--- a/cgraytracing_amd/csrc/cgrt_types.h
+++ b/cgraytracing_amd/csrc/cgrt_types.h
@@ -4,6 +4,7 @@
 #include <stdint.h>
 
 #include "cgrt_inside_sphere.h"
+#include "cgrt_unreachable_sphere.h"
 
 namespace cgrt {
 
@@ -156,6 +157,7 @@
     int32_t single_ray;
     int32_t light_hf_only;
     InsideTrait inside;
+    uint32_t reach;
 };
 
 }
diff --git a/cgraytracing_amd/csrc/cgrt_unreachable_sphere.h b/cgraytracing_amd/csrc/cgrt_unreachable_sphere.h
--- /dev/null
+++ b/cgraytracing_amd/csrc/cgrt_unreachable_sphere.h
@@ -0,0 +1,123 @@
+#ifndef CGRT_UNREACHABLE_SPHERE_H
+#define CGRT_UNREACHABLE_SPHERE_H
+#include <stdint.h>
+#include <cmath>
+
+#include "cgrt_inside_sphere.h"
+
+static constexpr int kUnreachSpheresMax = 32;
+static constexpr int kUnreachOccMax = 4;
+static constexpr double kUnreachRound = 8e-15;
+static constexpr double kUnreachEps = 1e-4;
+
+struct UnreachOccluder {
+    int32_t idx;
+    double c[3];
+    double r;
+    double cap;
+    double margin;
+};
+struct UnreachTrait {
+    int32_t n;
+    uint32_t reach;
+    int32_t n_occ;
+    UnreachOccluder occ[kUnreachOccMax];
+};
+
+inline bool unreach_special(double refl, double transp) { return !(refl < kUnreachEps) || !(transp < kUnreachEps); }
+inline double unreach_dist(const InsideBall &a, const InsideBall &b) {
+    const double dx = a.c[0] - b.c[0], dy = a.c[1] - b.c[1], dz = a.c[2] - b.c[2];
+    return sqrt(dx * dx + dy * dy + dz * dz);
+}
+inline double unreach_cap(const InsideBall *s, const double *refl, const double *transp, int n, int i) {
+    double far = sqrt(s[i].r2);
+    for (int k = 0; k < n; k++)
+        if (k != i && unreach_special(refl[k], transp[k])) far = fmax(far, unreach_dist(s[i], s[k]) + sqrt(s[k].r2));
+    return 4 * far;
+}
+inline double unreach_e(double cap) { return sqrt(kUnreachRound * (2 * cap) * (2 * cap)); }
+inline double unreach_m(double cap) { return cap * 1e-9 + 1e-6; }
+inline double unreach_origin_margin(double cap) { return 2 * unreach_e(cap) + unreach_m(cap); }
+inline double unreach_depth(double cap) { return 4 * unreach_e(cap) + unreach_m(cap); }
+inline double unreach_clearance(double cap) { return kUnreachEps + 8 * unreach_e(cap) + unreach_m(cap); }
+
+inline bool unreach_occludes(const InsideBall *s, const double *refl, const double *transp, int n, int i, double cap) {
+    if (unreach_special(refl[i], transp[i])) return false;
+    const double ri = sqrt(s[i].r2), clear = unreach_clearance(cap);
+    for (int k = 0; k < n; k++)
+        if (k != i && unreach_special(refl[k], transp[k]) && !(unreach_dist(s[i], s[k]) - ri - sqrt(s[k].r2) > clear)) return false;
+    return true;
+}
+inline bool unreach_nested(const InsideBall &bi, const InsideBall &bj, double cap) {
+    return sqrt(bi.r2) - unreach_dist(bi, bj) - sqrt(bj.r2) >= unreach_depth(cap);
+}
+
+inline UnreachTrait unreach_trait(const InsideBall *s, const double *refl, const double *transp, int n) {
+    UnreachTrait t{};
+    if (n < 1 || n > kUnreachSpheresMax) return t;
+    t.n = n;
+    t.reach = inside_full_mask(n);
+    for (int j = 0; j < n; j++)
+        if (!inside_finite(s[j]) || !(fabs(refl[j]) < 1e150) || !(fabs(transp[j]) < 1e150)) return t;
+    for (int j = 0; j < n; j++)
+        for (int k = j + 1; k < n; k++)
+            if (s[j].c[0] == s[k].c[0] && s[j].c[1] == s[k].c[1] && s[j].c[2] == s[k].c[2] && s[j].r2 == s[k].r2) return t;
+    double cap[kUnreachSpheresMax];
+    uint32_t occludes = 0u, hidden = 0u;
+    for (int i = 0; i < n; i++) {
+        cap[i] = unreach_cap(s, refl, transp, n, i);
+        if (unreach_occludes(s, refl, transp, n, i, cap[i])) occludes |= 1u << i;
+    }
+    for (int i = 0; i < n; i++)
+        for (int j = 0; j < n && ((occludes >> i) & 1u); j++)
+            if (j != i && unreach_nested(s[i], s[j], cap[i])) hidden |= 1u << j;
+    for (int i = 0; i < n && t.n_occ < kUnreachOccMax; i++) {
+        if (!((occludes >> i) & 1u) || ((hidden >> i) & 1u)) continue;
+        uint32_t hides = 0u;
+        for (int j = 0; j < n; j++)
+            if (j != i && unreach_nested(s[i], s[j], cap[i])) hides |= 1u << j;
+        if ((hides & t.reach) == 0u) continue;
+        t.reach &= ~hides;
+        UnreachOccluder &o = t.occ[t.n_occ++];
+        o.idx = i;
+        o.c[0] = s[i].c[0], o.c[1] = s[i].c[1], o.c[2] = s[i].c[2];
+        o.r = sqrt(s[i].r2);
+        o.cap = cap[i];
+        o.margin = unreach_origin_margin(cap[i]);
+    }
+    return t;
+}
+inline bool unreach_drops(const UnreachTrait &t) { return t.n > 0 && t.reach != inside_full_mask(t.n); }
+
+#ifdef CGRT_REACH_WALK
+static constexpr bool kReachWalk = true;
+#else
+static constexpr bool kReachWalk = false;
+#endif
+CGRT_INSIDE_HD uint32_t unreach_compact(uint32_t x, uint32_t mask) {
+    uint32_t out = 0u, k = 0u;
+    for (uint32_t m = mask; m != 0u; m &= m - 1u, k++) out |= ((x >> __builtin_ctz(m)) & 1u) << k;
+    return out;
+}
+CGRT_INSIDE_HD int unreach_compact_index(int i, uint32_t mask) { return __builtin_popcount(mask & ((1u << i) - 1u)); }
+
+inline bool unreach_launch_ok(const UnreachTrait &t, const double cam[3], double lens_radius) {
+    if (!unreach_drops(t)) return false;
+    const double R = lens_radius > 0 ? lens_radius : 0.0;
+    if (!(fabs(cam[0]) < 1e150 && fabs(cam[1]) < 1e150 && fabs(cam[2]) < 1e150 && R < 1e150)) return false;
+    const double lo[3] = {cam[0] - R, cam[1] - R, cam[2]}, hi[3] = {cam[0] + R, cam[1] + R, cam[2]};
+    for (int k = 0; k < t.n_occ; k++) {
+        const UnreachOccluder &o = t.occ[k];
+        double near2 = 0, far2 = 0;
+        for (int a = 0; a < 3; a++) {
+            const double gap = fmax(fmax(lo[a] - o.c[a], o.c[a] - hi[a]), 0.0), f = fmax(fabs(lo[a] - o.c[a]), fabs(hi[a] - o.c[a]));
+            near2 += gap * gap;
+            far2 += f * f;
+        }
+        const double out = o.r + o.margin;
+        if (!(near2 > out * out && far2 <= o.cap * o.cap)) return false;
+    }
+    return true;
+}
+
+#endif
diff --git a/cgraytracing_amd/unreachable.py b/cgraytracing_amd/unreachable.py
--- /dev/null
+++ b/cgraytracing_amd/unreachable.py
@@ -0,0 +1,32 @@
+import ctypes as C
+
+import numpy as np
+
+from . import _capi, engine
+from ._capi import check
+
+
+def unreachable_spheres(scene):
+    n, reach, n_occ, last = C.c_int32(), C.c_uint32(), C.c_int32(), C.c_uint32()
+    occ = np.zeros(8, np.int32)
+    check(scene._L.cgrt_scene_unreachable_spheres(scene._h, C.byref(n), C.byref(reach), occ.ctypes.data, 8, C.byref(n_occ), C.byref(last)))
+    return dict(n=n.value, reach=reach.value, occluders=[int(i) for i in occ[:n_occ.value]], last=last.value)
+
+
+def trace_grid_all_spheres(scene, width, height, spp=1, camera=None, max_depth=5, seed=12345, rows=None, row_offset=0, stripe=None,
+                           sample_offset=0, spp_total=None, out=None, counters=None, accumulate=False, **switches):
+    import torch
+
+    rows = height - row_offset if rows is None else rows
+    dev = torch.device("cuda", scene.device)
+    if out is None:
+        out = torch.zeros((rows, width, 3), dtype=torch.float32, device=dev)
+    nhit = torch.zeros((rows, width), dtype=torch.int32, device=dev)
+    if counters is None:
+        counters = torch.zeros((_capi.CGRT_NCOUNTERS,), dtype=torch.int64, device=dev)
+    assert out.is_contiguous() and out.dtype == torch.float32 and tuple(out.shape) == (rows, width, 3)
+    flags = (_capi.GRID_ACCUMULATE if accumulate else 0) | engine._grid_flags(**switches) | _capi.GRID_NO_UNREACHABLE
+    cc, g = scene._structs(camera, width, height, rows, spp, max_depth, seed, row_offset, stripe, sample_offset, spp_total, flags)
+    st = torch.cuda.current_stream(dev).cuda_stream
+    check(scene._L.cgrt_trace_grid(scene._h, C.byref(cc), C.byref(g), out.data_ptr(), nhit.data_ptr(), counters.data_ptr(), C.c_void_p(st)))
+    return out, nhit, counters
diff --git a/include/cgrt.h b/include/cgrt.h
--- a/include/cgrt.h
+++ b/include/cgrt.h
@@ -79,6 +79,7 @@
     CGRT_GRID_LENS_TABLE = 16777216,
     CGRT_GRID_NO_SURE_TILES = 262144,
     CGRT_GRID_NO_INSIDE_TRIPS = 33554432,
+    CGRT_GRID_NO_UNREACHABLE = 134217728,
     CGRT_GRID_POSED = 67108864,
     CGRT_GRID_HITPOINTS = 32,
     CGRT_GRID_SPLIT_SAMPLES = 4
@@ -399,6 +400,8 @@
 int cgrt_scene_last_lens_stage(const cgrt_scene *s, int64_t *lds_tiles, int64_t *area_tiles);
 int cgrt_scene_last_lens_table(const cgrt_scene *s, int64_t *entries, int64_t *capacity, int32_t *reused);
 int cgrt_scene_inside_spheres(const cgrt_scene *s, int32_t *index, uint32_t *mask, double *rin2, int32_t cap, int32_t *n);
+int cgrt_scene_unreachable_spheres(const cgrt_scene *s, int32_t *n, uint32_t *reach, int32_t *occluder, int32_t cap, int32_t *n_occ,
+                                   uint32_t *last);
 int cgrt_scene_last_eye_launches(const cgrt_scene *s, int32_t *rows, int64_t cap, int64_t *n);
 
 int cgrt_relay_start_host(int32_t k, int32_t chunk_spp, int32_t spp, int64_t cap, int32_t extent, int64_t n01, int64_t n012, int64_t n_tiles,
```

Result: faster. 126,500, median of 6 (+5.0%).
